# MisEty/X-SLAM

Hardware: AMD Instinct MI355X
Metric: fps XKinectFusion 512^3 TSDF 640x480 CSFD @1/2/4/8 GPU; HBM GB/s on integrate (higher is better)
Workload: dtype f32 (complex<f32> CSFD)

## Files before the change

include/xslam_amd_pipeline.h:

```cpp
#ifndef XSLAM_AMD_PIPELINE_H
#define XSLAM_AMD_PIPELINE_H
#include <stddef.h>
#include <stdint.h>
#ifdef __cplusplus
extern "C" {
#endif

int xs_host_double_complex_table(int op, long n, const float *a, const float *b, float *out);
int xs_host_complex_table(int op, long n, const float *a, const float *b, float *out);

int xs_flat_yaml_get(const char *yaml_text, const char *key, char *out, int capacity);

void xs_kf_set_stream(void *stream);
void *xs_kf_create(const char *yaml_text);
void *xs_kf_create_sharded(const char *yaml_text, int rank, int count, void (*collective)(void *user, int op, void *dev_ptr, long n),
                           void *user);
void xs_kf_shard_planes(void *kf, int *owned2, int *stored2);
void xs_kf_destroy(void *kf);
void xs_kf_set_gt_poses(void *kf, int n, const float *c2w32);
int xs_kf_process_frame(void *kf, const uint16_t *depth_dev, size_t step_bytes);
void xs_kf_hint_next_frame(void *kf, const uint16_t *depth_dev, size_t step_bytes);
int xs_kf_process_frame_host(void *kf, const uint16_t *depth_host);
uint16_t *xs_kf_ingest_buffer(void *kf);
void xs_kf_get_camera2volume(void *kf, float *out32);
int xs_kf_gauss_newton_terms(void *kf, const uint16_t *depth_dev, size_t step_bytes, const float *c2v32, double *out29);
int xs_kf_relocalize(void *kf, const uint16_t *depth_dev, size_t step_bytes, float *c2v32, int iterations, float damping, double *loss_out);
int xs_kf_relocalize_batch(void *kf, int frames, const uint16_t *const *depth_dev, size_t step_bytes, float *c2v32xF, int iterations, float damping,
                           double *loss_out, int *ok_out);
int xs_kf_pose_hessian_terms(void *kf, const uint16_t *depth_dev, size_t step_bytes, const float *c2v32, double *out29);
int xs_kf_relocalize_newton(void *kf, const uint16_t *depth_dev, size_t step_bytes, float *c2v32, int iterations, float damping, double *loss_out,
                            int *fallbacks_out);
int xs_kf_relocalize_newton_batch(void *kf, int frames, const uint16_t *const *depth_dev, size_t step_bytes, float *c2v32xF, int iterations,
                                  float damping, double *loss_out, int *ok_out, int *fallbacks_out);
int xs_host_newton_seeded_poses(const float *c2v32, float *R36x21, float *t12x21);
int xs_host_newton_step(const double *s29, double damping, float *c2v32);
int xs_kf_score_poses(void *kf, const uint16_t *depth_dev, size_t step_bytes, int poses, const float *c2v32xP, double *out2xP);
int xs_kf_relocalize_global(void *kf, const uint16_t *depth_dev, size_t step_bytes, int poses, const float *c2v32xP, int keep, int iterations,
                            float damping, float *best_c2v32, double *report8);
struct xs_view_opts;
int xs_kf_score_views(void *kf, int poses, const float *c2v32xP, const struct xs_view_opts *opts, int min_weight, unsigned *out4xP);
int xs_kf_next_best_view(void *kf, int poses, const float *c2v32xP, const struct xs_view_opts *opts, int min_weight, unsigned min_hits,
                         unsigned *out4xP);
int xs_kf_clearance_field(void *kf, int max_radius_vox, int unknown_blocks, int min_weight, uint16_t *host_out);
int xs_kf_reachable(void *kf, const float *start_c2v32_or_null, float radius_m, int snap_vox, int unknown_blocks, int min_weight, int P, const float *c2v32xP,
                    unsigned char *reachable, unsigned short *clear2);
int xs_kf_next_reachable_view(void *kf, int poses, const float *c2v32xP, const struct xs_view_opts *opts, int min_weight, unsigned min_hits, unsigned *out4xP,
                              float radius_m, int snap_vox, int unknown_blocks, unsigned char *reachable);
int xs_kf_travel(void *kf, const float *start_c2v32_or_null, float radius_m, int snap_vox, int unknown_blocks, int min_weight, float max_travel_m, int P,
                 const float *c2v32xP, unsigned char *reachable, unsigned short *clear2, unsigned short *travel3);
int xs_kf_path_to(void *kf, const float *start_c2v32_or_null, float radius_m, int snap_vox, int unknown_blocks, int min_weight, float max_travel_m,
                  const float *target_c2v32, int capacity, int *voxels3, float *points3, int *needed_out);
int xs_kf_next_view_by_travel(void *kf, int poses, const float *c2v32xP, const struct xs_view_opts *opts, int min_weight, unsigned min_hits, unsigned *out4xP,
                              float radius_m, int snap_vox, int unknown_blocks, float max_travel_m, float bias_m, unsigned short *travel3_out);
int xs_kf_frontiers(void *kf, int cell, unsigned long long min_size, int min_weight, int capacity, unsigned long long *records8, int *count_out);
int xs_kf_propose_views(void *kf, float radius_m, int start_snap_vox, int unknown_blocks, int min_weight, int cell, unsigned long long min_size,
                        int views_per_cluster, float standoff_m, int snap_vox, int capacity, float *c2v32xP_out, int *cluster_out, int *count_out);
long long xs_kf_relocalization_index_voxels(void *kf);
long long xs_kf_export_point_cloud(void *kf, int max_buffer, float *points_host, float *normals_host);
long long xs_kf_export_ply(void *kf, int max_buffer, const char *filename);
long long xs_kf_export_mesh(void *kf, int min_weight, long long vertex_capacity, long long triangle_capacity, float *vertices_host,
                            float *normals_host, float *vertex_im_host, unsigned long long *edge_keys_host, int *triangles_host,
                            long long *triangle_count, int *has_im);
long long xs_kf_export_mesh_ply(void *kf, const char *filename);
void xs_kf_synchronize(void *kf);

int xs_kf_frame_id(void *kf);
int xs_kf_num_poses(void *kf);
void xs_kf_get_world2camera(void *kf, int idx, float *out32);
float xs_kf_tranc_dist(void *kf);
long long xs_kf_last_updated_voxels(void *kf);
long long xs_kf_last_raycast_hits(void *kf);
int xs_kf_icp_log(void *kf, double *out, int capacity);

int xs_kf_download_volume(void *kf, float *value, int *weight, float *grad);
int xs_kf_download_map(void *kf, int which, int level, float *out);
void *xs_kf_volume_ptr(void *kf, int which, size_t *step_bytes);

void xs_kf_set_profiling(void *kf, int level);
void xs_kf_stage_times(void *kf, double *ms6, long long *calls6);
void xs_kf_cumulative_counters(void *kf, long long *updated, long long *hits);
void xs_kf_reset_stage_times(void *kf);
void xs_kf_icp_iteration_times(void *kf, double *us4, long long *calls4);
void xs_kf_tail_host_times(void *kf, double *us4, long long *frames);
void xs_kf_gn_times(void *kf, double *pass_us, long long *passes, double *kernel_ms, long long *kernel_calls, int reset);
void xs_kf_gn_poll_times(void *kf, double *poll_us, long long *poll_passes, int reset);
void xs_kf_set_gn_post_pose(void *kf, int on);
void xs_kf_debug_set_icp_sequence(void *kf, unsigned long long v);
void xs_kf_debug_fail_icp_iteration(void *kf, int n);
void xs_kf_debug_post_delay(void *kf, int min_us, int max_us);
void xs_kf_rebuild_sign_map(void *kf);
long long xs_kf_composite_bytes(void *kf);
void xs_kf_list_cover_counts(void *kf, long long *counts4);

long long xs_kf_volume_generation(void *kf);
int xs_kf_save_checkpoint(void *kf, const char *path);
int xs_kf_load_checkpoint(void *kf, const char *path);
int xs_kf_save_tsdf_volume(void *kf, const char *path);

int xs_kf_merge_volume(void *kf, const float *src_value, const int *src_weight, const float *src_grad, size_t src_step, const int *src_res,
                       float src_voxel_size, float src_tranc_dist, const double *T16, int min_weight, unsigned long long *written);
int xs_kf_merge_map(void *kf, void *other_kf, const double *T16, int min_weight, unsigned long long *written);
int xs_kf_merge_checkpoint(void *kf, const char *path, const double *T16, int min_weight, unsigned long long *written);
int xs_host_merge_affine(const double *T16, double dst_voxel_size, double src_voxel_size, float *out12);
int xs_host_map_transform(const double *c2v_this16, const double *c2v_other16, double *T16);
int xs_host_merge_tile_box(const float *xform12, const int *lo3, const int *hi3, const int *src_res, int *box6);

int xs_kf_align_map(void *kf, void *other_kf, const double *T16xN, int N, int iterations, double damping, int min_weight, float max_residual,
                    double *T16_out, double *report8, double *loss_history);
int xs_kf_align_checkpoint(void *kf, const char *path, const double *T16xN, int N, int iterations, double damping, int min_weight, float max_residual,
                           double *T16_out, double *report8, double *loss_history);
int xs_host_align_seeded_maps(const double *T16, double vs_this, double vs_other, float *out144);
int xs_host_align_step(const double *s29, double damping, double *T16);

void *xs_refshape_create(const char *yaml_text);
void xs_refshape_destroy(void *rs);
int xs_refshape_process_frame_host(void *rs, const uint16_t *depth_host);
int xs_refshape_process_frame(void *rs, const uint16_t *depth_dev, size_t step_bytes);
int xs_refshape_frame_id(void *rs);
void xs_refshape_get_world2camera(void *rs, int idx, float *out32);
int xs_refshape_download_volume(void *rs, float *value, int *weight, float *grad);
int xs_refshape_download_map(void *rs, int which, int level, float *out);
int xs_refshape_icp_log(void *rs, double *out, int capacity);
int xs_refshape_hessian(const uint16_t *depth_dev, size_t depth_step, int rows, int cols, const float *intr4, const int *res3, float voxel_size,
                        const float *Rv2c36, const float *tv2c12, float tranc_dist, const float *gt_dev, int with_volumes, float *out4,
                        float *volumes_host);
int xs_refshape_loss(const uint16_t *depth_dev, size_t depth_step, int rows, int cols, const float *intr4, const int *res3, float voxel_size,
                     const float *Rv2c9, const float *tv2c3, float tranc_dist, const float *gt_dev, int with_volumes, float *out2,
                     float *volumes_host);

#ifdef __cplusplus
}
#endif
#endif
```

x-slam_amd/host/device_array.hpp:

```cpp
#pragma once
#include "kernel_containers.hpp"
#include <atomic>
#include <cstdio>
#include <cstdlib>
#include <hip/hip_runtime_api.h>
#include <hip/hip_vector_types.h>
#include <utility>
#include <vector>

namespace xs_host {
inline void safe_call(hipError_t err, const char *msg = nullptr) {
    if (hipSuccess != err) {
        printf("HIP error(%s): %s\n", msg ? msg : "", hipGetErrorString(err));
        exit(-1);
    }
}
inline hipStream_t &current_stream() { static thread_local hipStream_t s = nullptr; return s; }
}
#define hipSafeCall(e) xs_host::safe_call((e), #e)

class DeviceMemory {
public:
    DeviceMemory() : data_(nullptr), sizeBytes_(0), refcount_(nullptr) {}
    ~DeviceMemory() { release(); }
    DeviceMemory(size_t sizeBytes_arg) : data_(nullptr), sizeBytes_(0), refcount_(nullptr) { create(sizeBytes_arg); }
    DeviceMemory(void *ptr_arg, size_t sizeBytes_arg) : data_(ptr_arg), sizeBytes_(sizeBytes_arg), refcount_(nullptr) {}
    DeviceMemory(const DeviceMemory &o) : data_(o.data_), sizeBytes_(o.sizeBytes_), refcount_(o.refcount_) { if (refcount_) refcount_->fetch_add(1); }
    DeviceMemory &operator=(const DeviceMemory &o) {
        if (this != &o) {
            if (o.refcount_) o.refcount_->fetch_add(1);
            release();
            data_ = o.data_; sizeBytes_ = o.sizeBytes_; refcount_ = o.refcount_;
        }
        return *this;
    }
    void create(size_t sizeBytes_arg) {
        if (sizeBytes_arg == sizeBytes_) return;
        if (sizeBytes_arg > 0) {
            if (data_) release();
            sizeBytes_ = sizeBytes_arg;
            hipSafeCall(hipMalloc(&data_, sizeBytes_));
            refcount_ = new std::atomic<int>(1);
        }
    }
    void release() {
        if (refcount_ && refcount_->fetch_sub(1) == 1) {
            delete refcount_;
            hipSafeCall(hipFree(data_));
        }
        data_ = nullptr; sizeBytes_ = 0; refcount_ = nullptr;
    }
    void copyTo(DeviceMemory &other) const {
        if (empty()) other.release();
        else {
            other.create(sizeBytes_);
            hipSafeCall(hipMemcpyAsync(other.data_, data_, sizeBytes_, hipMemcpyDeviceToDevice, xs_host::current_stream()));
            hipSafeCall(hipStreamSynchronize(xs_host::current_stream()));
        }
    }
    void upload(const void *host_ptr_arg, size_t sizeBytes_arg) {
        create(sizeBytes_arg);
        hipSafeCall(hipMemcpyAsync(data_, host_ptr_arg, sizeBytes_, hipMemcpyHostToDevice, xs_host::current_stream()));
        hipSafeCall(hipStreamSynchronize(xs_host::current_stream()));
    }
    bool upload(const void *host_ptr_arg, std::size_t device_begin_byte_offset, std::size_t num_bytes) {
        if (device_begin_byte_offset + num_bytes > sizeBytes_) return false;
        hipSafeCall(hipMemcpyAsync((char *)data_ + device_begin_byte_offset, host_ptr_arg, num_bytes, hipMemcpyHostToDevice, xs_host::current_stream()));
        hipSafeCall(hipStreamSynchronize(xs_host::current_stream()));
        return true;
    }
    void download(void *host_ptr_arg) const {
        hipSafeCall(hipMemcpyAsync(host_ptr_arg, data_, sizeBytes_, hipMemcpyDeviceToHost, xs_host::current_stream()));
        hipSafeCall(hipStreamSynchronize(xs_host::current_stream()));
    }
    bool download(void *host_ptr_arg, std::size_t device_begin_byte_offset, std::size_t num_bytes) const {
        if (device_begin_byte_offset + num_bytes > sizeBytes_) return false;
        hipSafeCall(hipMemcpyAsync(host_ptr_arg, (const char *)data_ + device_begin_byte_offset, num_bytes, hipMemcpyDeviceToHost, xs_host::current_stream()));
        hipSafeCall(hipStreamSynchronize(xs_host::current_stream()));
        return true;
    }
    void swap(DeviceMemory &o) { std::swap(data_, o.data_); std::swap(sizeBytes_, o.sizeBytes_); std::swap(refcount_, o.refcount_); }
    template <class T> T *ptr() { return (T *)data_; }
    template <class T> const T *ptr() const { return (const T *)data_; }
    template <class U> operator PtrSz<U>() const { PtrSz<U> r; r.data = (U *)ptr<U>(); r.size = sizeBytes_ / sizeof(U); return r; }
    bool empty() const { return !data_; }
    size_t sizeBytes() const { return sizeBytes_; }

private:
    void *data_;
    std::size_t sizeBytes_;
    std::atomic<int> *refcount_;
};

class DeviceMemory2D {
public:
    DeviceMemory2D() : data_(nullptr), step_(0), colsBytes_(0), rows_(0), refcount_(nullptr) {}
    ~DeviceMemory2D() { release(); }
    DeviceMemory2D(int rows_arg, int colsBytes_arg) : data_(nullptr), step_(0), colsBytes_(0), rows_(0), refcount_(nullptr) { create(rows_arg, colsBytes_arg); }
    DeviceMemory2D(int rows_arg, int colsBytes_arg, void *data_arg, size_t step_arg)
        : data_(data_arg), step_(step_arg), colsBytes_(colsBytes_arg), rows_(rows_arg), refcount_(nullptr) {}
    DeviceMemory2D(const DeviceMemory2D &o) : data_(o.data_), step_(o.step_), colsBytes_(o.colsBytes_), rows_(o.rows_), refcount_(o.refcount_) {
        if (refcount_) refcount_->fetch_add(1);
    }
    DeviceMemory2D &operator=(const DeviceMemory2D &o) {
        if (this != &o) {
            if (o.refcount_) o.refcount_->fetch_add(1);
            release();
            colsBytes_ = o.colsBytes_; rows_ = o.rows_; data_ = o.data_; step_ = o.step_; refcount_ = o.refcount_;
        }
        return *this;
    }
    void create(int rows_arg, int colsBytes_arg) {
        if (colsBytes_ == colsBytes_arg && rows_ == rows_arg) return;
        if (rows_arg > 0 && colsBytes_arg > 0) {
            if (data_) release();
            colsBytes_ = colsBytes_arg; rows_ = rows_arg;
            step_ = ((size_t)colsBytes_ + 255) / 256 * 256;
            hipSafeCall(hipMalloc(&data_, step_ * (size_t)rows_));
            refcount_ = new std::atomic<int>(1);
        }
    }
    void release() {
        if (refcount_ && refcount_->fetch_sub(1) == 1) {
            delete refcount_;
            hipSafeCall(hipFree(data_));
        }
        colsBytes_ = 0; rows_ = 0; data_ = nullptr; step_ = 0; refcount_ = nullptr;
    }
    void copyTo(DeviceMemory2D &other) const {
        if (empty()) other.release();
        else {
            other.create(rows_, colsBytes_);
            hipSafeCall(hipMemcpy2DAsync(other.data_, other.step_, data_, step_, colsBytes_, rows_, hipMemcpyDeviceToDevice, xs_host::current_stream()));
            hipSafeCall(hipStreamSynchronize(xs_host::current_stream()));
        }
    }
    void upload(const void *host_ptr_arg, std::size_t host_step_arg, int rows_arg, int colsBytes_arg) {
        create(rows_arg, colsBytes_arg);
        hipSafeCall(hipMemcpy2DAsync(data_, step_, host_ptr_arg, host_step_arg, colsBytes_, rows_, hipMemcpyHostToDevice, xs_host::current_stream()));
        hipSafeCall(hipStreamSynchronize(xs_host::current_stream()));
    }
    void download(void *host_ptr_arg, std::size_t host_step_arg) const {
        hipSafeCall(hipMemcpy2DAsync(host_ptr_arg, host_step_arg, data_, step_, colsBytes_, rows_, hipMemcpyDeviceToHost, xs_host::current_stream()));
        hipSafeCall(hipStreamSynchronize(xs_host::current_stream()));
    }
    void swap(DeviceMemory2D &o) {
        std::swap(data_, o.data_); std::swap(step_, o.step_); std::swap(colsBytes_, o.colsBytes_); std::swap(rows_, o.rows_); std::swap(refcount_, o.refcount_);
    }
    template <class T> T *ptr(int y_arg = 0) { return (T *)((char *)data_ + y_arg * step_); }
    template <class T> const T *ptr(int y_arg = 0) const { return (const T *)((const char *)data_ + y_arg * step_); }
    template <class U> operator PtrStep<U>() const { PtrStep<U> r; r.data = (U *)ptr<U>(); r.step = step_; return r; }
    template <class U> operator PtrStepSz<U>() const {
        PtrStepSz<U> r; r.data = (U *)ptr<U>(); r.step = step_; r.cols = colsBytes_ / sizeof(U); r.rows = rows_; return r;
    }
    bool empty() const { return !data_; }
    int colsBytes() const { return colsBytes_; }
    int rows() const { return rows_; }
    size_t step() const { return step_; }

private:
    void *data_;
    std::size_t step_;
    int colsBytes_;
    int rows_;
    std::atomic<int> *refcount_;
};

template <class T>
class DeviceArray : public DeviceMemory {
public:
    using type = T;
    enum { elem_size = sizeof(T) };
    DeviceArray() {}
    DeviceArray(std::size_t size) : DeviceMemory(size * elem_size) {}
    DeviceArray(T *ptr, std::size_t size) : DeviceMemory(ptr, size * elem_size) {}
    DeviceArray(const DeviceArray &other) : DeviceMemory(other) {}
    DeviceArray &operator=(const DeviceArray &other) { DeviceMemory::operator=(other); return *this; }
    void create(std::size_t size) { DeviceMemory::create(size * elem_size); }
    void release() { DeviceMemory::release(); }
    void copyTo(DeviceArray &other) const { DeviceMemory::copyTo(other); }
    void upload(const T *host_ptr, std::size_t size) { DeviceMemory::upload(host_ptr, size * elem_size); }
    bool upload(const T *host_ptr, std::size_t device_begin_offset, std::size_t num_elements) {
        return DeviceMemory::upload(host_ptr, device_begin_offset * elem_size, num_elements * elem_size);
    }
    void download(T *host_ptr) const { DeviceMemory::download(host_ptr); }
    bool download(T *host_ptr, std::size_t device_begin_offset, std::size_t num_elements) const {
        return DeviceMemory::download(host_ptr, device_begin_offset * elem_size, num_elements * elem_size);
    }
    template <class A> void upload(const std::vector<T, A> &data) { upload(&data[0], data.size()); }
    template <typename A> void download(std::vector<T, A> &data) const { data.resize(size()); if (!data.empty()) download(&data[0]); }
    void swap(DeviceArray &other_arg) { DeviceMemory::swap(other_arg); }
    T *ptr() { return DeviceMemory::ptr<T>(); }
    const T *ptr() const { return DeviceMemory::ptr<T>(); }
    operator T *() { return ptr(); }
    operator const T *() const { return ptr(); }
    std::size_t size() const { return sizeBytes() / elem_size; }
};

template <class T>
class DeviceArray2D : public DeviceMemory2D {
public:
    using type = T;
    enum { elem_size = sizeof(T) };
    DeviceArray2D() {}
    DeviceArray2D(int rows, int cols) : DeviceMemory2D(rows, cols * elem_size) {}
    DeviceArray2D(int rows, int cols, void *data, std::size_t stepBytes) : DeviceMemory2D(rows, cols * elem_size, data, stepBytes) {}
    DeviceArray2D(const DeviceArray2D &other) : DeviceMemory2D(other) {}
    DeviceArray2D &operator=(const DeviceArray2D &other) { DeviceMemory2D::operator=(other); return *this; }
    void create(int rows, int cols) { DeviceMemory2D::create(rows, cols * elem_size); }
    void release() { DeviceMemory2D::release(); }
    void copyTo(DeviceArray2D &other) const { DeviceMemory2D::copyTo(other); }
    void upload(const void *host_ptr, std::size_t host_step, int rows, int cols) { DeviceMemory2D::upload(host_ptr, host_step, rows, cols * elem_size); }
    void download(void *host_ptr, std::size_t host_step) const { DeviceMemory2D::download(host_ptr, host_step); }
    void swap(DeviceArray2D &other_arg) { DeviceMemory2D::swap(other_arg); }
    template <class A> void upload(const std::vector<T, A> &data, int cols) { upload(&data[0], cols * elem_size, data.size() / cols, cols); }
    template <class A> void download(std::vector<T, A> &data, int &elem_step) const {
        elem_step = cols();
        data.resize(cols() * rows());
        if (!data.empty()) download(&data[0], colsBytes());
    }
    T *ptr(int y = 0) { return DeviceMemory2D::ptr<T>(y); }
    const T *ptr(int y = 0) const { return DeviceMemory2D::ptr<T>(y); }
    operator T *() { return ptr(); }
    operator const T *() const { return ptr(); }
    int cols() const { return DeviceMemory2D::colsBytes() / elem_size; }
    int rows() const { return DeviceMemory2D::rows(); }
    std::size_t elem_step() const { return DeviceMemory2D::step() / elem_size; }
};
```

x-slam_amd/host/xs_launchers.hpp:

```cpp
#pragma once
#include "../../include/xslam_amd.h"
#include "xs_types.hpp"
#include "host_algebra.hpp"

namespace xs_host {
inline void check_rc(int rc, const char *what) {
    if (rc != 0) {
        printf("HIP error(%s): %s\n", what, xs_last_error());
        exit(-1);
    }
}
inline void sync() { hipSafeCall(hipStreamSynchronize(current_stream())); }
struct Scratch {
    DeviceArray<unsigned char> icp_ws, reduce_ws, integrate_ws;
    DeviceArray<double> sums;
    DeviceArray<float> ray_ws;
    static Scratch &get() { static thread_local Scratch s; return s; }
    void *icp() {
        if (icp_ws.size() != xs_icp_workspace_bytes()) {
            icp_ws.create(xs_icp_workspace_bytes());
            check_rc(xs_icp_workspace_init(icp_ws.ptr(), current_stream()), "icp workspace");
        }
        return icp_ws.ptr();
    }
    void *integrate(const int *res) {
        const size_t bytes = xs_integrate_workspace_bytes(res, res[2]);
        if (integrate_ws.size() != bytes) integrate_ws.create(bytes);
        return integrate_ws.ptr();
    }
    float *ray(int rows, int cols) { if (ray_ws.size() != (size_t)rows * cols) ray_ws.create((size_t)rows * cols); return ray_ws.ptr(); }
    void *reduce() {
        if (reduce_ws.size() != xs_tsdf_reduce_workspace_bytes()) {
            reduce_ws.create(xs_tsdf_reduce_workspace_bytes());
            check_rc(xs_tsdf_reduce_workspace_init(reduce_ws.ptr(), current_stream()), "reduce workspace");
        }
        return reduce_ws.ptr();
    }
    double *sum_buf() { if (sums.size() != 64) sums.create(64); return sums.ptr(); }
};
}

inline void initVolume(PtrStep<short> , PtrStep<float> value_volume,
                       PtrStep<int> weight_volume, PtrStep<float> grad_volume, const int3 &volume_resolution) {
    const int res[3] = {volume_resolution.x, volume_resolution.y, volume_resolution.z};
    xs_host::check_rc(xs_init_volume(value_volume.data, weight_volume.data, grad_volume.data, value_volume.step, res, 0, res[2],
                                     xs_host::current_stream()), "initVolume");
    xs_host::sync();
}

inline void integrateTsdfVolume(const PtrStepSz<ushort> &depth, const Intr &intr, int max_weight, const int3 &volume_resolution,
                                float voxel_size, const MatS33 &Rv2c, const devComplex3 &tv2c, const devComplex3 & ,
                                float tranc_dist, PtrStep<float> value_volume, PtrStep<int> weight_volume, PtrStep<float> grad_volume,
                                DeviceArray2D<float> &depthScaled, int , float threshold = 0.0f, float  = 0.0f,
                                unsigned long long *updated_dev = nullptr, bool synchronise = true) {
    depthScaled.create(depth.rows, depth.cols);
    const int res[3] = {volume_resolution.x, volume_resolution.y, volume_resolution.z};
    hipStream_t st = xs_host::current_stream();
    xs_host::check_rc(xs_scale_depth(depth.data, depth.step, depth.rows, depth.cols, depthScaled.ptr(), depthScaled.step(), st), "scaleDepth");
    xs_host::check_rc(xs_integrate_scaled(depthScaled.ptr(), depthScaled.step(), depth.rows, depth.cols, &intr.fx, max_weight, res, voxel_size,
                                          &Rv2c.data[0].x.re, &tv2c.x.re, tranc_dist, value_volume.data, weight_volume.data, grad_volume.data,
                                          value_volume.step, threshold, 0, res[2], updated_dev, nullptr, xs_host::Scratch::get().integrate(res), st),
                      "integrateTsdfVolume");
    if (synchronise) xs_host::sync();
}

inline void raycast(const Intr &intr, const MatS33 &Rc2v, const devComplex3 &tc2v, const MatS33 &Rv2w, const devComplex3 &tv2w,
                    float tranc_dist, const int3 &volume_resolution, float voxel_size, const PtrStep<float> &value_volume,
                    const PtrStep<float> &grad_volume, MapArr &vmap, MapArr &nmap, unsigned long long *hits_dev = nullptr,
                    float *workspace = nullptr, xs_raycast_opts *opts = nullptr) {
    const int res[3] = {volume_resolution.x, volume_resolution.y, volume_resolution.z};
    xs_host::check_rc(xs_raycast_ex(&intr.fx, &Rc2v.data[0].x.re, &tc2v.x.re, &Rv2w.data[0].x.re, &tv2w.x.re, tranc_dist, res, voxel_size,
                                    value_volume.data, grad_volume.data, value_volume.step, &vmap.ptr()->re, &nmap.ptr()->re, vmap.step(),
                                    vmap.rows() / 3, vmap.cols(), hits_dev, workspace ? workspace : xs_host::Scratch::get().ray(vmap.rows() / 3, vmap.cols()), opts,
                                    xs_host::current_stream()), "raycast");
}

inline void estimateCombined(const MatS33 &Rcurr, const devComplex3 &tcurr, const MapArr &vmap_curr, const MapArr &nmap_curr,
                             const MatS33 &Rprev_inv, const devComplex3 &tprev, const Intr &intr, const MapArr &vmap_g_prev,
                             const MapArr &nmap_g_prev, float distThres, float angleThres, DeviceArray2D<devComplexICP> & ,
                             DeviceArray<devComplexICP> & , hostComplexICP *matrixA_host, hostComplexICP *vectorB_host,
                             long long *inliers = nullptr) {
    auto &S = xs_host::Scratch::get();
    xs_host::check_rc(xs_estimate_combined(&Rcurr.data[0].x.re, &tcurr.x.re, &vmap_curr.ptr()->re, &nmap_curr.ptr()->re,
                                           &Rprev_inv.data[0].x.re, &tprev.x.re, &intr.fx, &vmap_g_prev.ptr()->re, &nmap_g_prev.ptr()->re,
                                           vmap_curr.step(), vmap_curr.rows() / 3, vmap_curr.cols(), distThres, angleThres, S.icp(),
                                           nullptr , reinterpret_cast<double *>(matrixA_host), reinterpret_cast<double *>(vectorB_host),
                                           inliers, xs_host::current_stream()), "estimateCombined");
}

inline void bilateralFilter(const DeviceArray2D<ushort> &src, MapArr &dst) {
    xs_host::check_rc(xs_bilateral_filter(src.ptr(), src.step(), src.rows(), src.cols(), &dst.ptr()->re, dst.step(), xs_host::current_stream()), "bilateralFilter");
}
inline void pyrDown(const MapArr &src, MapArr &dst) {
    dst.create(src.rows() / 2, src.cols() / 2);
    xs_host::check_rc(xs_pyr_down(&src.ptr()->re, src.step(), src.rows(), src.cols(), &dst.ptr()->re, dst.step(), xs_host::current_stream()), "pyrDown");
}
inline void createVMap(const Intr &intr, const MapArr &depth, MapArr &vmap) {
    vmap.create(depth.rows() * 3, depth.cols());
    xs_host::check_rc(xs_create_vmap(&intr.fx, &depth.ptr()->re, depth.step(), depth.rows(), depth.cols(), &vmap.ptr()->re, vmap.step(), xs_host::current_stream()), "createVMap");
}
inline void createNMap(const MapArr &vmap, MapArr &nmap) {
    nmap.create(vmap.rows(), vmap.cols());
    xs_host::check_rc(xs_create_nmap(&vmap.ptr()->re, &nmap.ptr()->re, vmap.step(), vmap.rows() / 3, vmap.cols(), xs_host::current_stream()), "createNMap");
}
inline void resizeVMap(const MapArr &input, MapArr &output, bool synchronise = true) {
    output.create((input.rows() / 3 / 2) * 3, input.cols() / 2);
    xs_host::check_rc(xs_resize_vmap(&input.ptr()->re, input.step(), input.rows() / 3, input.cols(), &output.ptr()->re, output.step(), xs_host::current_stream()), "resizeVMap");
    if (synchronise) xs_host::sync();
}
inline void resizeNMap(const MapArr &input, MapArr &output, bool synchronise = true) {
    output.create((input.rows() / 3 / 2) * 3, input.cols() / 2);
    xs_host::check_rc(xs_resize_nmap(&input.ptr()->re, input.step(), input.rows() / 3, input.cols(), &output.ptr()->re, output.step(), xs_host::current_stream()), "resizeNMap");
    if (synchronise) xs_host::sync();
}

inline float4 ComputeLocalTsdf_hessian(const PtrStepSz<ushort> &depth, const Intr &intr, DeviceArray2D<float> &depthScaled,
                                        const int3 &volume_resolution, float voxel_size, const MatD33 &Rv2c, const devDComplex3 &tv2c,
                                        float tranc_dist, float , float , DeviceArray<float> &gt_vec,
                                        DeviceArray<float> &real_vec, DeviceArray<float> &grad_vec, DeviceArray<float> &hessian_vec,
                                        DeviceArray<int> &count_vec) {
    depthScaled.create(depth.rows, depth.cols);
    const int res[3] = {volume_resolution.x, volume_resolution.y, volume_resolution.z};
    auto &S = xs_host::Scratch::get();
    hipStream_t st = xs_host::current_stream();
    xs_host::check_rc(xs_scale_depth(depth.data, depth.step, depth.rows, depth.cols, depthScaled.ptr(), depthScaled.step(), st), "scaleDepth");
    const bool vols = !real_vec.empty() && !grad_vec.empty() && !hessian_vec.empty() && !count_vec.empty();
    xs_host::check_rc(xs_compute_local_tsdf_hessian(depthScaled.ptr(), depthScaled.step(), depth.rows, depth.cols, &intr.fx, res, voxel_size,
                                                    &Rv2c.data[0].x.re_re, &tv2c.x.re_re, tranc_dist, gt_vec.ptr(),
                                                    vols ? real_vec.ptr() : nullptr, vols ? grad_vec.ptr() : nullptr,
                                                    vols ? hessian_vec.ptr() : nullptr, vols ? count_vec.ptr() : nullptr, 0, res[2],
                                                    S.reduce(), S.sum_buf(), st), "ComputeLocalTsdf_hessian");
    double h[4];
    hipSafeCall(hipMemcpyAsync(h, S.sum_buf(), sizeof(h), hipMemcpyDeviceToHost, st));
    xs_host::sync();
    return float4{(float)h[0], (float)h[1], (float)h[2], (float)h[3]};
}
inline float2 ComputeLocalTsdf_loss(const PtrStepSz<ushort> &depth, const Intr &intr, DeviceArray2D<float> &depthScaled,
                                     const int3 &volume_resolution, float voxel_size, const Mat33 &Rv2c, const float3 &tv2c,
                                     float tranc_dist, float , float , DeviceArray<float> &gt_vec,
                                     DeviceArray<float> &real_vec, DeviceArray<int> &count_vec) {
    depthScaled.create(depth.rows, depth.cols);
    const int res[3] = {volume_resolution.x, volume_resolution.y, volume_resolution.z};
    auto &S = xs_host::Scratch::get();
    hipStream_t st = xs_host::current_stream();
    xs_host::check_rc(xs_scale_depth(depth.data, depth.step, depth.rows, depth.cols, depthScaled.ptr(), depthScaled.step(), st), "scaleDepth");
    const bool vols = !real_vec.empty() && !count_vec.empty();
    xs_host::check_rc(xs_compute_local_tsdf_loss(depthScaled.ptr(), depthScaled.step(), depth.rows, depth.cols, &intr.fx, res, voxel_size,
                                                 &Rv2c.data[0].x, &tv2c.x, tranc_dist, gt_vec.ptr(), vols ? real_vec.ptr() : nullptr,
                                                 vols ? count_vec.ptr() : nullptr, 0, res[2], S.reduce(), S.sum_buf(), st), "ComputeLocalTsdf_loss");
    double h[2];
    hipSafeCall(hipMemcpyAsync(h, S.sum_buf(), sizeof(h), hipMemcpyDeviceToHost, st));
    xs_host::sync();
    return float2{(float)h[0], (float)h[1]};
}

inline size_t extractPoints(const PtrStep<float> &value_volume, const PtrStep<int> & , const PtrStep<float> & ,
                            const int3 &volume_resolution, float voxel_size, PtrSz<float3> output, int zs0 = 0, int z0 = 0, int z1 = -1) {
    const int res[3] = {volume_resolution.x, volume_resolution.y, volume_resolution.z};
    static thread_local DeviceArray<unsigned char> ws;
    if (ws.size() < xs_extract_workspace_bytes(res)) ws.create(xs_extract_workspace_bytes(res));
    size_t count = 0;
    xs_host::check_rc(xs_extract_points(value_volume.data, value_volume.step, res, voxel_size, zs0, z0, z1 < 0 ? res[2] - 1 : z1,
                                        reinterpret_cast<float *>(output.data), output.size, ws.ptr(), &count, nullptr, xs_host::current_stream()),
                      "extractPoints");
    return count;
}
inline void extractNormals(const PtrStep<float> &value_volume, const PtrStep<int> & , const PtrStep<float> & ,
                           const int3 &volume_resolution, float voxel_size, PtrSz<float3> points, PtrSz<float3> normal, int zs0 = 0, int zs1 = -1) {
    const int res[3] = {volume_resolution.x, volume_resolution.y, volume_resolution.z};
    xs_host::check_rc(xs_extract_normals(value_volume.data, value_volume.step, res, voxel_size, zs0, zs1 < 0 ? res[2] : zs1,
                                         reinterpret_cast<const float *>(points.data), points.size, reinterpret_cast<float *>(normal.data),
                                         xs_host::current_stream()), "extractNormals");
    xs_host::sync();
}
```

x-slam_amd/pipeline.py:

```python
import collections
import ctypes as C
import os

import numpy as np

from . import capi

_HERE = os.path.dirname(os.path.abspath(__file__))
LIB_PATH = os.path.join(_HERE, "libxslam_host.so")
if not os.path.exists(LIB_PATH):
    raise ImportError(f"{LIB_PATH} not found: run __graft_entry__.build() (make -C x-slam_amd/host). There is no CPU fallback.")
_lib = C.CDLL(LIB_PATH)

_vp, _sz = C.c_void_p, C.c_size_t
_f32p, _f64p, _i32p = C.POINTER(C.c_float), C.POINTER(C.c_double), C.POINTER(C.c_int)
COLLECTIVE_CB = C.CFUNCTYPE(None, C.c_void_p, C.c_int, C.c_void_p, C.c_long)
_SIGS = {
    "xs_kf_create_sharded": (_vp, [C.c_char_p, C.c_int, C.c_int, COLLECTIVE_CB, _vp]),
    "xs_kf_shard_planes": (None, [_vp, _i32p, _i32p]),
    "xs_host_double_complex_table": (C.c_int, [C.c_int, C.c_long, _f32p, _f32p, _f32p]),
    "xs_host_complex_table": (C.c_int, [C.c_int, C.c_long, _f32p, _f32p, _f32p]),
    "xs_flat_yaml_get": (C.c_int, [C.c_char_p, C.c_char_p, C.c_char_p, C.c_int]),
    "xs_kf_set_stream": (None, [_vp]),
    "xs_kf_create": (_vp, [C.c_char_p]),
    "xs_kf_destroy": (None, [_vp]),
    "xs_kf_set_gt_poses": (None, [_vp, C.c_int, _f32p]),
    "xs_kf_process_frame": (C.c_int, [_vp, _vp, _sz]),
    "xs_kf_process_frame_host": (C.c_int, [_vp, _vp]),
    "xs_kf_ingest_buffer": (_vp, [_vp]),
    "xs_kf_get_camera2volume": (None, [_vp, _f32p]),
    "xs_kf_gauss_newton_terms": (C.c_int, [_vp, _vp, _sz, _f32p, _f64p]),
    "xs_kf_relocalize": (C.c_int, [_vp, _vp, _sz, _f32p, C.c_int, C.c_float, _f64p]),
    "xs_kf_relocalize_batch": (C.c_int, [_vp, C.c_int, C.POINTER(_vp), _sz, _f32p, C.c_int, C.c_float, _f64p, _i32p]),
    "xs_kf_pose_hessian_terms": (C.c_int, [_vp, _vp, _sz, _f32p, _f64p]),
    "xs_kf_relocalize_newton": (C.c_int, [_vp, _vp, _sz, _f32p, C.c_int, C.c_float, _f64p, _i32p]),
    "xs_kf_relocalize_newton_batch": (C.c_int, [_vp, C.c_int, C.POINTER(_vp), _sz, _f32p, C.c_int, C.c_float, _f64p, _i32p, _i32p]),
    "xs_host_newton_seeded_poses": (C.c_int, [_f32p, _f32p, _f32p]),
    "xs_host_newton_step": (C.c_int, [_f64p, C.c_double, _f32p]),
    "xs_kf_score_poses": (C.c_int, [_vp, _vp, _sz, C.c_int, _f32p, _f64p]),
    "xs_kf_relocalize_global": (C.c_int, [_vp, _vp, _sz, C.c_int, _f32p, C.c_int, C.c_int, C.c_float, _f32p, _f64p]),
    "xs_kf_score_views": (C.c_int, [_vp, C.c_int, _f32p, C.POINTER(capi.ViewOpts), C.c_int, C.POINTER(C.c_uint)]),
    "xs_kf_next_best_view": (C.c_int, [_vp, C.c_int, _f32p, C.POINTER(capi.ViewOpts), C.c_int, C.c_uint, C.POINTER(C.c_uint)]),
    "xs_kf_clearance_field": (C.c_int, [_vp, C.c_int, C.c_int, C.c_int, C.POINTER(C.c_uint16)]),
    "xs_kf_reachable": (C.c_int, [_vp, _f32p, C.c_float, C.c_int, C.c_int, C.c_int, C.c_int, _f32p, C.POINTER(C.c_ubyte), C.POINTER(C.c_uint16)]),
    "xs_kf_next_reachable_view": (C.c_int, [_vp, C.c_int, _f32p, C.POINTER(capi.ViewOpts), C.c_int, C.c_uint, C.POINTER(C.c_uint), C.c_float, C.c_int,
                                            C.c_int, C.POINTER(C.c_ubyte)]),
    "xs_kf_travel": (C.c_int, [_vp, _f32p, C.c_float, C.c_int, C.c_int, C.c_int, C.c_float, C.c_int, _f32p, C.POINTER(C.c_ubyte), C.POINTER(C.c_uint16),
                               C.POINTER(C.c_uint16)]),
    "xs_kf_path_to": (C.c_int, [_vp, _f32p, C.c_float, C.c_int, C.c_int, C.c_int, C.c_float, _f32p, C.c_int, _i32p, _f32p, _i32p]),
    "xs_kf_next_view_by_travel": (C.c_int, [_vp, C.c_int, _f32p, C.POINTER(capi.ViewOpts), C.c_int, C.c_uint, C.POINTER(C.c_uint), C.c_float, C.c_int,
                                            C.c_int, C.c_float, C.c_float, C.POINTER(C.c_uint16)]),
    "xs_kf_frontiers": (C.c_int, [_vp, C.c_int, C.c_ulonglong, C.c_int, C.c_int, C.POINTER(C.c_uint64), _i32p]),
    "xs_kf_propose_views": (C.c_int, [_vp, C.c_float, C.c_int, C.c_int, C.c_int, C.c_int, C.c_ulonglong, C.c_int, C.c_float, C.c_int, C.c_int, _f32p, _i32p,
                                      _i32p]),
    "xs_kf_relocalization_index_voxels": (C.c_longlong, [_vp]),
    "xs_kf_export_point_cloud": (C.c_longlong, [_vp, C.c_int, _f32p, _f32p]),
    "xs_kf_export_ply": (C.c_longlong, [_vp, C.c_int, C.c_char_p]),
    "xs_kf_export_mesh": (C.c_longlong, [_vp, C.c_int, C.c_longlong, C.c_longlong, _f32p, _f32p, _f32p, C.POINTER(C.c_uint64), _i32p,
                                         C.POINTER(C.c_longlong), _i32p]),
    "xs_kf_export_mesh_ply": (C.c_longlong, [_vp, C.c_char_p]),
    "xs_kf_synchronize": (None, [_vp]),
    "xs_kf_frame_id": (C.c_int, [_vp]),
    "xs_kf_num_poses": (C.c_int, [_vp]),
    "xs_kf_get_world2camera": (None, [_vp, C.c_int, _f32p]),
    "xs_kf_tranc_dist": (C.c_float, [_vp]),
    "xs_kf_last_updated_voxels": (C.c_longlong, [_vp]),
    "xs_kf_last_raycast_hits": (C.c_longlong, [_vp]),
    "xs_kf_icp_log": (C.c_int, [_vp, _f64p, C.c_int]),
    "xs_kf_download_volume": (C.c_int, [_vp, _f32p, _i32p, _f32p]),
    "xs_kf_download_map": (C.c_int, [_vp, C.c_int, C.c_int, _f32p]),
    "xs_kf_volume_ptr": (_vp, [_vp, C.c_int, C.POINTER(_sz)]),
    "xs_kf_set_profiling": (None, [_vp, C.c_int]),
    "xs_kf_stage_times": (None, [_vp, _f64p, C.POINTER(C.c_longlong)]),
    "xs_kf_reset_stage_times": (None, [_vp]),
    "xs_kf_icp_iteration_times": (None, [_vp, _f64p, C.POINTER(C.c_longlong)]),
    "xs_kf_tail_host_times": (None, [_vp, _f64p, C.POINTER(C.c_longlong)]),
    "xs_kf_set_gn_post_pose": (None, [_vp, C.c_int]),
    "xs_kf_gn_poll_times": (None, [_vp, _f64p, C.POINTER(C.c_longlong), C.c_int]),
    "xs_kf_gn_times": (None, [_vp, _f64p, C.POINTER(C.c_longlong), _f64p, C.POINTER(C.c_longlong), C.c_int]),
    "xs_kf_debug_set_icp_sequence": (None, [_vp, C.c_ulonglong]),
    "xs_kf_debug_fail_icp_iteration": (None, [_vp, C.c_int]),
    "xs_kf_debug_post_delay": (None, [_vp, C.c_int, C.c_int]),
    "xs_kf_composite_bytes": (C.c_longlong, [_vp]),
    "xs_kf_rebuild_sign_map": (None, [_vp]),
    "xs_kf_hint_next_frame": (None, [_vp, _vp, _sz]),
    "xs_kf_list_cover_counts": (None, [_vp, C.POINTER(C.c_longlong)]),
    "xs_kf_cumulative_counters": (None, [_vp, C.POINTER(C.c_longlong), C.POINTER(C.c_longlong)]),
    "xs_kf_volume_generation": (C.c_longlong, [_vp]),
    "xs_kf_save_checkpoint": (C.c_int, [_vp, C.c_char_p]),
    "xs_kf_load_checkpoint": (C.c_int, [_vp, C.c_char_p]),
    "xs_kf_save_tsdf_volume": (C.c_int, [_vp, C.c_char_p]),
    "xs_kf_merge_volume": (C.c_int, [_vp, _vp, _vp, _vp, _sz, _i32p, C.c_float, C.c_float, _f64p, C.c_int, C.POINTER(C.c_ulonglong)]),
    "xs_kf_merge_map": (C.c_int, [_vp, _vp, _f64p, C.c_int, C.POINTER(C.c_ulonglong)]),
    "xs_kf_merge_checkpoint": (C.c_int, [_vp, C.c_char_p, _f64p, C.c_int, C.POINTER(C.c_ulonglong)]),
    "xs_host_merge_affine": (C.c_int, [_f64p, C.c_double, C.c_double, _f32p]),
    "xs_host_map_transform": (C.c_int, [_f64p, _f64p, _f64p]),
    "xs_host_merge_tile_box": (C.c_int, [_f32p, _i32p, _i32p, _i32p, _i32p]),
    "xs_kf_align_map": (C.c_int, [_vp, _vp, _f64p, C.c_int, C.c_int, C.c_double, C.c_int, C.c_float, _f64p, _f64p, _f64p]),
    "xs_kf_align_checkpoint": (C.c_int, [_vp, C.c_char_p, _f64p, C.c_int, C.c_int, C.c_double, C.c_int, C.c_float, _f64p, _f64p, _f64p]),
    "xs_host_align_seeded_maps": (C.c_int, [_f64p, C.c_double, C.c_double, _f32p]),
    "xs_host_align_step": (C.c_int, [_f64p, C.c_double, _f64p]),
    "xs_refshape_create": (_vp, [C.c_char_p]),
    "xs_refshape_destroy": (None, [_vp]),
    "xs_refshape_process_frame_host": (C.c_int, [_vp, _vp]),
    "xs_refshape_process_frame": (C.c_int, [_vp, _vp, _sz]),
    "xs_refshape_frame_id": (C.c_int, [_vp]),
    "xs_refshape_get_world2camera": (None, [_vp, C.c_int, _f32p]),
    "xs_refshape_download_volume": (C.c_int, [_vp, _f32p, _i32p, _f32p]),
    "xs_refshape_download_map": (C.c_int, [_vp, C.c_int, C.c_int, _f32p]),
    "xs_refshape_icp_log": (C.c_int, [_vp, _f64p, C.c_int]),
    "xs_refshape_hessian": (C.c_int, [_vp, _sz, C.c_int, C.c_int, _f32p, _i32p, C.c_float, _f32p, _f32p, C.c_float, _vp, C.c_int, _f32p, _f32p]),
    "xs_refshape_loss": (C.c_int, [_vp, _sz, C.c_int, C.c_int, _f32p, _i32p, C.c_float, _f32p, _f32p, C.c_float, _vp, C.c_int, _f32p, _f32p]),
}
for _n, (_r, _a) in _SIGS.items():
    _f = getattr(_lib, _n)
    _f.restype, _f.argtypes = _r, _a

STAGES = ("surface", "icp", "scale", "integrate", "raycast", "resize")
MAPS = {"depths_curr": 0, "vmaps_curr": 1, "nmaps_curr": 2, "vmaps_g_prev": 3, "nmaps_g_prev": 4}


def yaml_text(params: dict) -> str:
    out = []
    for k, v in params.items():
        if isinstance(v, bool):
            v = "true" if v else "false"
        elif isinstance(v, float):
            v = repr(float(np.float32(v))) if abs(v) < 1e-3 and v != 0 else repr(v)
        out.append(f"{k}: {v}")
    return "\n".join(out) + "\n"


HDC_OPS = {"add": 0, "sub": 1, "mul": 2, "div": 3, "sqrt": 4, "abs": 5, "exp": 6, "log": 7, "sin": 8, "cos": 9, "pow": 10, "f1": 11,
           "conj": 12, "norm": 13, "cmp": 14}


def host_double_complex(op, a, b=None):
    a = np.ascontiguousarray(a, dtype=np.float32).reshape(-1, 4)
    b = a if b is None else np.ascontiguousarray(b, dtype=np.float32).reshape(-1, 4)
    out = np.empty_like(a)
    rc = _lib.xs_host_double_complex_table(HDC_OPS[op], a.shape[0], a.ctypes.data_as(_f32p), b.ctypes.data_as(_f32p), out.ctypes.data_as(_f32p))
    if rc != 0:
        raise ValueError("bad op")
    return out


def host_complex(op_code, a, b=None):
    a = np.ascontiguousarray(a, dtype=np.float32).reshape(-1, 2)
    b = a if b is None else np.ascontiguousarray(b, dtype=np.float32).reshape(-1, 2)
    out = np.empty_like(a)
    rc = _lib.xs_host_complex_table(int(op_code), a.shape[0], a.ctypes.data_as(_f32p), b.ctypes.data_as(_f32p), out.ctypes.data_as(_f32p))
    if rc != 0:
        raise ValueError("bad op")
    return out


def host_newton_seeded_poses(c2v):
    m = np.ascontiguousarray(c2v, dtype=np.float32).reshape(32)
    R, t = np.zeros((21, 3, 3, 4), np.float32), np.zeros((21, 3, 4), np.float32)
    _lib.xs_host_newton_seeded_poses(m.ctypes.data_as(_f32p), R.ctypes.data_as(_f32p), t.ctypes.data_as(_f32p))
    return R, t


def host_newton_step(s29, damping, c2v):
    s = np.ascontiguousarray(s29, dtype=np.float64).reshape(29)
    m = np.ascontiguousarray(c2v, dtype=np.float32).reshape(32).copy()
    rc = _lib.xs_host_newton_step(s.ctypes.data_as(_f64p), float(damping), m.ctypes.data_as(_f32p))
    return rc == 0, m.reshape(4, 4, 2)


def _real44(m):
    a = np.asarray(m, dtype=np.float64)
    if a.shape == (4, 4, 2):
        a = a[..., 0]
    return np.ascontiguousarray(a.reshape(4, 4))


def merge_affine(T, dst_voxel_size, src_voxel_size):
    t = _real44(T)
    out = np.zeros(12, np.float32)
    if _lib.xs_host_merge_affine(t.ctypes.data_as(_f64p), float(dst_voxel_size), float(src_voxel_size), out.ctypes.data_as(_f32p)) != 0:
        raise ValueError("merge_affine: an input is not finite, or a voxel size is not positive")
    return out


def map_transform(c2v_this, c2v_other):
    a, b = _real44(c2v_this), _real44(c2v_other)
    out = np.zeros((4, 4), np.float64)
    _lib.xs_host_map_transform(a.ctypes.data_as(_f64p), b.ctypes.data_as(_f64p), out.ctypes.data_as(_f64p))
    return out


def align_seeded_maps(T, vs_this, vs_other):
    t = _real44(T)
    out = np.zeros((6, 12, 2), np.float32)
    if _lib.xs_host_align_seeded_maps(t.ctypes.data_as(_f64p), float(vs_this), float(vs_other), out.ctypes.data_as(_f32p)) != 0:
        raise ValueError("align_seeded_maps: an input is not finite, or a voxel size is not positive")
    return out


def align_step(s29, damping, T):
    s = np.ascontiguousarray(s29, dtype=np.float64).reshape(29)
    t = _real44(T).copy()
    rc = _lib.xs_host_align_step(s.ctypes.data_as(_f64p), float(damping), t.ctypes.data_as(_f64p))
    return rc == 0, t


def merge_tile_box(xform12, lo, hi, src_res):
    m = np.ascontiguousarray(xform12, np.float32).reshape(12)
    l, h, s = (np.ascontiguousarray(a, np.int32).reshape(3) for a in (lo, hi, src_res))
    box = np.zeros(6, np.int32)
    rc = _lib.xs_host_merge_tile_box(m.ctypes.data_as(_f32p), l.ctypes.data_as(_i32p), h.ctypes.data_as(_i32p), s.ctypes.data_as(_i32p), box.ctypes.data_as(_i32p))
    return (box[:3].copy(), box[3:].copy()) if rc == 1 else None


def _halton(i, base):
    f, r = 1.0, 0.0
    while i > 0:
        f /= base
        r += f * (i % base)
        i //= base
    return r


def _se3_exp(xi):
    v, w = np.asarray(xi[:3], np.float64), np.asarray(xi[3:], np.float64)
    th = float(np.linalg.norm(w))
    K = np.array([[0.0, -w[2], w[1]], [w[2], 0.0, -w[0]], [-w[1], w[0], 0.0]])
    if th < 1e-12:
        R, V = np.eye(3) + K, np.eye(3) + K
    else:
        R = np.eye(3) + np.sin(th) / th * K + (1 - np.cos(th)) / th ** 2 * K @ K
        V = np.eye(3) + (1 - np.cos(th)) / th ** 2 * K + (th - np.sin(th)) / th ** 3 * K @ K
    T = np.eye(4)
    T[:3, :3], T[:3, 3] = R, V @ v
    return T


POSE_CANDIDATE_PRIMES = (2, 3, 5, 7, 11, 13)


def pose_candidates(center_c2v, box_t, box_r, n):
    c = np.asarray(center_c2v, np.float64)
    c = c[..., 0] if c.ndim == 3 else c
    assert c.shape == (4, 4)
    out = np.zeros((int(n), 4, 4, 2), np.float32)
    for i in range(int(n)):
        u = np.array([2.0 * _halton(i + 1, b) - 1.0 for b in POSE_CANDIDATE_PRIMES])
        out[i, ..., 0] = c @ _se3_exp(np.concatenate([u[:3] * float(box_t), u[3:] * float(box_r)]))
    return out


def flat_yaml_get(text, key):
    buf = C.create_string_buffer(1024)
    n = _lib.xs_flat_yaml_get(text.encode(), key.encode(), buf, 1024)
    return None if n < 0 else buf.value.decode()


def set_stream(stream):
    _lib.xs_kf_set_stream(None if stream is None else (stream.cuda_stream if hasattr(stream, "cuda_stream") else int(stream)))


class Mesh(collections.namedtuple("Mesh", "vertices vertex_im normals triangles edge_keys")):
    """A triangle mesh of the TSDF (KinectFusion.export_mesh): numpy arrays, vertices in ascending edge key."""


class KinectFusion:

    def __init__(self, params, gt_poses=None):
        text = params if isinstance(params, str) else yaml_text(params)
        self.cfg = {}
        for line in text.splitlines():
            if ":" in line:
                k, v = line.split(":", 1)
                self.cfg[k.strip()] = v.split("#")[0].strip()
        self.h = _lib.xs_kf_create(text.encode())
        if not self.h:
            raise ValueError("xs_kf_create failed (missing config key, or a retired one set?)")
        self.res = [int(self.cfg[f"tsdf_size_{a}"]) for a in "xyz"]
        self.width, self.height = int(self.cfg["depth_width"]), int(self.cfg["depth_height"])
        if gt_poses is not None:
            g = np.ascontiguousarray(gt_poses, dtype=np.float32).reshape(-1, 32)
            _lib.xs_kf_set_gt_poses(self.h, g.shape[0], g.ctypes.data_as(_f32p))

    def close(self):
        if getattr(self, "h", None) and _lib is not None:
            _lib.xs_kf_destroy(self.h)
            self.h = None

    def __del__(self):
        self.close()

    def process_frame(self, depth_dev, step_bytes=None):
        ptr = depth_dev if isinstance(depth_dev, int) else depth_dev.data_ptr()
        step = step_bytes if step_bytes is not None else self.width * 2
        return _lib.xs_kf_process_frame(self.h, ptr, step)

    def hint_next_frame(self, depth_dev, step_bytes=None):
        _lib.xs_kf_hint_next_frame(self.h, depth_dev.data_ptr(), step_bytes or self.width * 2)

    def process_frame_host(self, depth_u16):
        d = np.ascontiguousarray(depth_u16, dtype=np.uint16)
        return _lib.xs_kf_process_frame_host(self.h, d.ctypes.data)

    def ingest_buffer(self):
        ptr = _lib.xs_kf_ingest_buffer(self.h)
        n = self.width * self.height
        return np.ctypeslib.as_array((C.c_uint16 * n).from_address(ptr)).reshape(self.height, self.width)

    def camera2volume(self):
        out = np.zeros(32, np.float32)
        _lib.xs_kf_get_camera2volume(self.h, out.ctypes.data_as(_f32p))
        return out.reshape(4, 4, 2)

    def gauss_newton_terms(self, depth_dev, c2v):
        m = np.ascontiguousarray(c2v, dtype=np.float32).reshape(32)
        out = np.zeros(29, np.float64)
        ok = _lib.xs_kf_gauss_newton_terms(self.h, depth_dev.data_ptr(), self.width * 2, m.ctypes.data_as(_f32p), out.ctypes.data_as(_f64p))
        return out if ok == 1 else None

    def pose_hessian_terms(self, depth_dev, c2v):
        m = np.ascontiguousarray(c2v, dtype=np.float32).reshape(32)
        out = np.zeros(29, np.float64)
        ok = _lib.xs_kf_pose_hessian_terms(self.h, depth_dev.data_ptr(), self.width * 2, m.ctypes.data_as(_f32p), out.ctypes.data_as(_f64p))
        return out if ok == 1 else None

    def pose_hessian(self, depth_dev, c2v):
        s = self.pose_hessian_terms(depth_dev, c2v)
        if s is None:
            return None
        H = np.zeros((6, 6))
        H[np.triu_indices(6)] = s[:21]
        H = H + np.triu(H, 1).T
        return H, s[21:27].copy(), float(s[27]), int(s[28])

    def relocalize(self, depth_dev, c2v, iterations=5, damping=1e-3, method="gauss_newton"):
        m = np.ascontiguousarray(c2v, dtype=np.float32).reshape(32).copy()
        hist = np.zeros(iterations + 1, np.float64)
        if method == "newton":
            fb = C.c_int(0)
            ok = _lib.xs_kf_relocalize_newton(self.h, depth_dev.data_ptr(), self.width * 2, m.ctypes.data_as(_f32p), iterations, damping,
                                              hist.ctypes.data_as(_f64p), C.cast(C.byref(fb), _i32p))
            return ok == 1, m.reshape(4, 4, 2), hist, int(fb.value)
        if method != "gauss_newton":
            raise ValueError(f"relocalize: unknown method {method!r}")
        ok = _lib.xs_kf_relocalize(self.h, depth_dev.data_ptr(), self.width * 2, m.ctypes.data_as(_f32p), iterations, damping,
                                   hist.ctypes.data_as(_f64p))
        return ok == 1, m.reshape(4, 4, 2), hist

    def relocalize_batch(self, depths, c2vs, iterations=5, damping=1e-3, method="gauss_newton"):
        F = len(depths)
        m = np.ascontiguousarray(c2vs, dtype=np.float32).reshape(F * 32).copy()
        hist = np.zeros((F, iterations + 1), np.float64)
        ok = np.zeros(F, np.int32)
        P = (_vp * max(F, 1))(*[d if isinstance(d, int) else d.data_ptr() for d in depths])
        if method == "newton":
            fb = np.zeros(max(F, 1), np.int32)
            n = _lib.xs_kf_relocalize_newton_batch(self.h, F, P, self.width * 2, m.ctypes.data_as(_f32p), iterations, damping,
                                                   hist.ctypes.data_as(_f64p), ok.ctypes.data_as(_i32p), fb.ctypes.data_as(_i32p))
            if n < 0:
                raise ValueError("xs_kf_relocalize_newton_batch: bad arguments")
            return ok == 1, m.reshape(F, 4, 4, 2), hist, fb[:F]
        if method != "gauss_newton":
            raise ValueError(f"relocalize_batch: unknown method {method!r}")
        n = _lib.xs_kf_relocalize_batch(self.h, F, P, self.width * 2, m.ctypes.data_as(_f32p), iterations, damping, hist.ctypes.data_as(_f64p),
                                        ok.ctypes.data_as(_i32p))
        if n < 0:
            raise ValueError("xs_kf_relocalize_batch: bad arguments")
        return ok == 1, m.reshape(F, 4, 4, 2), hist

    def score_poses(self, depth_dev, c2vs):
        m = np.ascontiguousarray(c2vs, dtype=np.float32).reshape(-1)
        P = m.size // 32
        assert m.size == 32 * P
        out = np.zeros((max(P, 1), 2), np.float64)
        rc = _lib.xs_kf_score_poses(self.h, depth_dev.data_ptr(), self.width * 2, P, m.ctypes.data_as(_f32p), out.ctypes.data_as(_f64p))
        if rc != 1:
            raise ValueError("xs_kf_score_poses: bad arguments" if rc < 0 else "xs_kf_score_poses: no volume")
        return out[:P, 0].copy(), out[:P, 1].copy()

    def relocalize_global(self, depth_dev, candidates, keep=8, iterations=10, damping=1e-3):
        m = np.ascontiguousarray(candidates, dtype=np.float32).reshape(-1)
        P = m.size // 32
        assert m.size == 32 * P and P > 0
        best = m[:32].copy()
        rep = np.zeros(8, np.float64)
        rc = _lib.xs_kf_relocalize_global(self.h, depth_dev.data_ptr(), self.width * 2, P, m.ctypes.data_as(_f32p), int(keep), int(iterations),
                                          float(damping), best.ctypes.data_as(_f32p), rep.ctypes.data_as(_f64p))
        if rc < 0:
            raise ValueError("xs_kf_relocalize_global: bad arguments")
        report = dict(index=int(rep[0]), S_before=float(rep[1]), S_after=float(rep[2]), sum_loss_after=float(rep[3]), count_after=float(rep[4]),
                      refined_ok=int(rep[5]), index_voxels=int(rep[6]))
        return rc == 1, best.reshape(4, 4, 2), report

    @staticmethod
    def _view_call(name, rc, bad):
        if rc == -2:
            raise capi.XsError(f"{name}: not available in shard mode (occlusion along a ray is not additive over z-slabs)")
        if rc == bad:
            raise ValueError(f"{name}: bad arguments or options")

    def score_views(self, c2vs, rays=(80, 60), t_near=0.2, t_far=5.0, step=None, min_weight=1):
        m = np.ascontiguousarray(c2vs, dtype=np.float32).reshape(-1)
        P = m.size // 32
        assert m.size == 32 * P
        out = np.zeros((max(P, 1), 4), np.uint32)
        opts = capi.view_opts(rays, t_near, t_far, step)
        rc = _lib.xs_kf_score_views(self.h, P, m.ctypes.data_as(_f32p), C.byref(opts), int(min_weight), out.ctypes.data_as(C.POINTER(C.c_uint)))
        self._view_call("xs_kf_score_views", rc, -1)
        if rc != 1:
            raise ValueError("xs_kf_score_views: no volume")
        return out[:P].copy()

    def next_best_view(self, candidates, min_hits=None, rays=(80, 60), t_near=0.2, t_far=5.0, step=None, min_weight=1):
        m = np.ascontiguousarray(candidates, dtype=np.float32).reshape(-1)
        P = m.size // 32
        assert m.size == 32 * P
        if min_hits is None:
            min_hits = int(rays[0]) * int(rays[1]) // 4
        out = np.zeros((max(P, 1), 4), np.uint32)
        opts = capi.view_opts(rays, t_near, t_far, step)
        rc = _lib.xs_kf_next_best_view(self.h, P, m.ctypes.data_as(_f32p), C.byref(opts), int(min_weight), int(min_hits),
                                       out.ctypes.data_as(C.POINTER(C.c_uint)))
        self._view_call("xs_kf_next_best_view", rc, -3)
        return int(rc), out[:P].copy()

    def clearance_field(self, max_radius_vox=8, unknown_blocks=True, min_weight=1):
        out = np.zeros((self.res[2], self.res[1], self.res[0]), np.uint16)
        rc = _lib.xs_kf_clearance_field(self.h, int(max_radius_vox), int(bool(unknown_blocks)), int(min_weight), out.ctypes.data_as(C.POINTER(C.c_uint16)))
        self._reach_call("xs_kf_clearance_field", rc, -1)
        if rc != 1:
            raise ValueError("xs_kf_clearance_field: no volume")
        return out

    @staticmethod
    def _reach_call(name, rc, bad):
        if rc == -2:
            raise capi.XsError(f"{name}: not available in shard mode (distance and connectivity are not additive over z-slabs)")
        if rc == bad:
            raise ValueError(f"{name}: bad arguments or options")

    def reachable(self, c2vs, radius_m, start=None, snap_vox=4, unknown_blocks=True, min_weight=1):
        m = np.ascontiguousarray(c2vs, dtype=np.float32).reshape(-1)
        P = m.size // 32
        assert m.size == 32 * P
        flags, clear2 = np.zeros(max(P, 1), np.uint8), np.zeros(max(P, 1), np.uint16)
        s = None if start is None else np.ascontiguousarray(start, dtype=np.float32).reshape(32)
        rc = _lib.xs_kf_reachable(self.h, None if s is None else s.ctypes.data_as(_f32p), float(radius_m), int(snap_vox), int(bool(unknown_blocks)),
                                  int(min_weight), P, m.ctypes.data_as(_f32p), flags.ctypes.data_as(C.POINTER(C.c_ubyte)),
                                  clear2.ctypes.data_as(C.POINTER(C.c_uint16)))
        self._reach_call("xs_kf_reachable", rc, -1)
        if rc != 1:
            raise ValueError("xs_kf_reachable: no volume")
        return flags[:P].astype(bool), clear2[:P].copy()

    def next_reachable_view(self, candidates, radius_m, min_hits=None, rays=(80, 60), t_near=0.2, t_far=5.0, step=None, min_weight=1, snap_vox=4,
                            unknown_blocks=True):
        m = np.ascontiguousarray(candidates, dtype=np.float32).reshape(-1)
        P = m.size // 32
        assert m.size == 32 * P
        if min_hits is None:
            min_hits = int(rays[0]) * int(rays[1]) // 4
        out, flags = np.zeros((max(P, 1), 4), np.uint32), np.zeros(max(P, 1), np.uint8)
        opts = capi.view_opts(rays, t_near, t_far, step)
        rc = _lib.xs_kf_next_reachable_view(self.h, P, m.ctypes.data_as(_f32p), C.byref(opts), int(min_weight), int(min_hits),
                                            out.ctypes.data_as(C.POINTER(C.c_uint)), float(radius_m), int(snap_vox), int(bool(unknown_blocks)),
                                            flags.ctypes.data_as(C.POINTER(C.c_ubyte)))
        self._reach_call("xs_kf_next_reachable_view", rc, -3)
        return int(rc), out[:P].copy(), flags[:P].astype(bool)

    def _travel_m(self, units):
        vs = float(np.float32(float(self.cfg["tsdf_voxel_size"])))
        u = np.asarray(units, np.uint16)
        return np.where(u == capi.TRAVEL_NONE, np.inf, u.astype(np.float64) * vs / 3.0)

    def travel(self, c2vs, radius_m, start=None, snap_vox=4, unknown_blocks=True, min_weight=1, max_travel_m=None):
        m = np.ascontiguousarray(c2vs, dtype=np.float32).reshape(-1)
        P = m.size // 32
        assert m.size == 32 * P
        flags, clear2, cost = np.zeros(max(P, 1), np.uint8), np.zeros(max(P, 1), np.uint16), np.zeros(max(P, 1), np.uint16)
        s = None if start is None else np.ascontiguousarray(start, dtype=np.float32).reshape(32)
        rc = _lib.xs_kf_travel(self.h, None if s is None else s.ctypes.data_as(_f32p), float(radius_m), int(snap_vox), int(bool(unknown_blocks)),
                               int(min_weight), 0.0 if max_travel_m is None else float(max_travel_m), P, m.ctypes.data_as(_f32p),
                               flags.ctypes.data_as(C.POINTER(C.c_ubyte)), clear2.ctypes.data_as(C.POINTER(C.c_uint16)),
                               cost.ctypes.data_as(C.POINTER(C.c_uint16)))
        self._reach_call("xs_kf_travel", rc, -1)
        if rc != 1:
            raise ValueError("xs_kf_travel: no volume")
        return flags[:P].astype(bool), clear2[:P].copy(), self._travel_m(cost[:P])

    def path_to(self, c2v, radius_m, start=None, snap_vox=4, unknown_blocks=True, min_weight=1, max_travel_m=None, capacity=1024):
        t = np.ascontiguousarray(c2v, dtype=np.float32).reshape(32)
        s = None if start is None else np.ascontiguousarray(start, dtype=np.float32).reshape(32)
        capacity = max(int(capacity), 1)
        for _ in range(2):
            voxels, points, needed = np.zeros((capacity, 3), np.int32), np.zeros((capacity, 3), np.float32), C.c_int(0)
            rc = _lib.xs_kf_path_to(self.h, None if s is None else s.ctypes.data_as(_f32p), float(radius_m), int(snap_vox), int(bool(unknown_blocks)),
                                    int(min_weight), 0.0 if max_travel_m is None else float(max_travel_m), t.ctypes.data_as(_f32p), capacity,
                                    voxels.ctypes.data_as(_i32p), points.ctypes.data_as(_f32p), C.byref(needed))
            if rc != -4:
                break
            capacity = int(needed.value)
        self._reach_call("xs_kf_path_to", rc, -1)
        if rc < 0:
            raise capi.XsError(f"xs_kf_path_to: {rc}")
        return None if rc == 0 else (points[:rc].copy(), voxels[:rc].copy())

    def next_view_by_travel(self, candidates, radius_m, bias_m=0.5, min_hits=None, rays=(80, 60), t_near=0.2, t_far=5.0, step=None, min_weight=1,
                            snap_vox=4, unknown_blocks=True, max_travel_m=None):
        m = np.ascontiguousarray(candidates, dtype=np.float32).reshape(-1)
        P = m.size // 32
        assert m.size == 32 * P
        if min_hits is None:
            min_hits = int(rays[0]) * int(rays[1]) // 4
        out, cost = np.zeros((max(P, 1), 4), np.uint32), np.zeros(max(P, 1), np.uint16)
        opts = capi.view_opts(rays, t_near, t_far, step)
        rc = _lib.xs_kf_next_view_by_travel(self.h, P, m.ctypes.data_as(_f32p), C.byref(opts), int(min_weight), int(min_hits),
                                            out.ctypes.data_as(C.POINTER(C.c_uint)), float(radius_m), int(snap_vox), int(bool(unknown_blocks)),
                                            0.0 if max_travel_m is None else float(max_travel_m), float(bias_m), cost.ctypes.data_as(C.POINTER(C.c_uint16)))
        self._reach_call("xs_kf_next_view_by_travel", rc, -3)
        return int(rc), out[:P].copy(), self._travel_m(cost[:P])

    FRONTIER_DTYPE = np.dtype([("label", np.uint32), ("count", np.uint64), ("sum", np.uint64, 3), ("centroid", np.float32, 3), ("min", np.int32, 3),
                               ("max", np.int32, 3)])

    @staticmethod
    def _frontier_call(name, rc):
        if rc == -2:
            raise capi.XsError(f"{name}: not available in shard mode (neither connectivity nor a cluster is additive over z-slabs)")
        if rc == -1:
            raise ValueError(f"{name}: bad arguments or options")

    def frontiers(self, cell_vox=32, min_size=8, min_weight=1):
        capacity, n = 1024, C.c_int(0)
        for _ in range(2):
            rec = np.zeros((max(capacity, 1), capi.FRONTIER_RECORD_WORDS), np.uint64)
            rc = _lib.xs_kf_frontiers(self.h, int(cell_vox), int(min_size), int(min_weight), capacity, rec.ctypes.data_as(C.POINTER(C.c_uint64)), C.byref(n))
            if rc != -4:
                break
            capacity = int(n.value)
        self._frontier_call("xs_kf_frontiers", rc)
        if rc != 1:
            raise ValueError("xs_kf_frontiers: no volume" if rc == 0 else f"xs_kf_frontiers: {rc}")
        rec = rec[:n.value]
        out = np.zeros(len(rec), self.FRONTIER_DTYPE)
        out["label"], out["count"], out["sum"] = rec[:, 0], rec[:, 1], rec[:, 2:5]
        vs = np.float32(float(self.cfg["tsdf_voxel_size"]))
        q = (rec[:, 2:5].astype(np.float64) / np.maximum(rec[:, 1:2], 1).astype(np.float64)).astype(np.float32)
        out["centroid"] = (q + np.float32(0.5)) * vs
        for name, col in (("min", 5), ("max", 6)):
            out[name] = np.stack([(rec[:, col] >> np.uint64(s)) & np.uint64(0xFFFF) for s in (0, 16, 32)], axis=1).astype(np.int32)
        return out

    def propose_views(self, radius_m, views_per_cluster=6, standoff_m=1.0, cell_vox=32, min_size=8, snap_vox=4, start_snap_vox=4, unknown_blocks=True,
                      min_weight=1):
        capacity, n = 1024, C.c_int(0)
        for _ in range(2):
            m, idx = np.zeros((max(capacity, 1), 4, 4, 2), np.float32), np.zeros(max(capacity, 1), np.int32)
            rc = _lib.xs_kf_propose_views(self.h, float(radius_m), int(start_snap_vox), int(bool(unknown_blocks)), int(min_weight), int(cell_vox), int(min_size),
                                          int(views_per_cluster), float(standoff_m), int(snap_vox), capacity, m.ctypes.data_as(_f32p), idx.ctypes.data_as(_i32p),
                                          C.byref(n))
            if rc != -4:
                break
            capacity = int(n.value)
        self._frontier_call("xs_kf_propose_views", rc)
        if rc != 1:
            raise ValueError("xs_kf_propose_views: no volume" if rc == 0 else f"xs_kf_propose_views: {rc}")
        return m[:n.value].copy(), idx[:n.value].copy()

    def explore_step(self, radius_m, views_per_cluster=6, standoff_m=1.0, cell_vox=32, min_size=8, snap_vox=4, unknown_blocks=True, min_weight=1, bias_m=0.5,
                     min_hits=None, rays=(80, 60), t_near=0.2, t_far=5.0, step=None, max_travel_m=None):
        cands, cluster = self.propose_views(radius_m, views_per_cluster, standoff_m, cell_vox, min_size, snap_vox, snap_vox, unknown_blocks, min_weight)
        if len(cands) == 0:
            return None
        pick, counts, travel_m = self.next_view_by_travel(cands, radius_m, bias_m=bias_m, min_hits=min_hits, rays=rays, t_near=t_near, t_far=t_far, step=step,
                                                          min_weight=min_weight, snap_vox=snap_vox, unknown_blocks=unknown_blocks, max_travel_m=max_travel_m)
        if pick < 0:
            return None
        path = self.path_to(cands[pick], radius_m, snap_vox=snap_vox, unknown_blocks=unknown_blocks, min_weight=min_weight, max_travel_m=max_travel_m)
        return dict(index=pick, pose=cands[pick].copy(), cluster=int(cluster[pick]), counts=counts[pick].copy(), travel_m=float(travel_m[pick]), path=path)

    def relocalization_index_voxels(self):
        return int(_lib.xs_kf_relocalization_index_voxels(self.h))

    def export_point_cloud(self, max_buffer=1000000):
        p = np.zeros((max_buffer, 3), np.float32)
        nr = np.zeros((max_buffer, 3), np.float32)
        n = _lib.xs_kf_export_point_cloud(self.h, max_buffer, p.ctypes.data_as(_f32p), nr.ctypes.data_as(_f32p))
        return p[:n], nr[:n]

    def export_ply(self, filename, max_buffer=1000000):
        return _lib.xs_kf_export_ply(self.h, max_buffer, str(filename).encode())

    def export_mesh(self, min_weight=1):
        nt, has_im = C.c_longlong(0), C.c_int(0)
        nv = _lib.xs_kf_export_mesh(self.h, min_weight, 0, 0, None, None, None, None, None, C.byref(nt), C.byref(has_im))
        while True:
            cap_v, cap_t = nv, nt.value
            v, n, im = (np.zeros((cap_v, 3), np.float32) for _ in range(3))
            k = np.zeros(cap_v, np.uint64)
            t = np.zeros((cap_t, 3), np.int32)
            nv = _lib.xs_kf_export_mesh(self.h, min_weight, cap_v, cap_t, v.ctypes.data_as(_f32p), n.ctypes.data_as(_f32p), im.ctypes.data_as(_f32p),
                                        k.ctypes.data_as(C.POINTER(C.c_uint64)), t.ctypes.data_as(_i32p), C.byref(nt), C.byref(has_im))
            if nv <= cap_v and nt.value <= cap_t:
                return Mesh(v[:nv], im[:nv] if has_im.value else None, n[:nv], t[:nt.value], k[:nv])

    def export_mesh_ply(self, filename):
        return _lib.xs_kf_export_mesh_ply(self.h, str(filename).encode())

    def synchronize(self):
        _lib.xs_kf_synchronize(self.h)

    @property
    def frame_id(self):
        return _lib.xs_kf_frame_id(self.h)

    def num_poses(self):
        return _lib.xs_kf_num_poses(self.h)

    def world2camera(self, idx=-1):
        out = np.zeros(32, np.float32)
        _lib.xs_kf_get_world2camera(self.h, idx, out.ctypes.data_as(_f32p))
        return out.reshape(4, 4, 2)

    def tranc_dist(self):
        return _lib.xs_kf_tranc_dist(self.h)

    def last_U(self):
        return _lib.xs_kf_last_updated_voxels(self.h)

    def last_hits(self):
        return _lib.xs_kf_last_raycast_hits(self.h)

    def icp_log(self):
        n = _lib.xs_kf_icp_log(self.h, None, 0)
        out = np.zeros(n, np.float64)
        if n:
            _lib.xs_kf_icp_log(self.h, out.ctypes.data_as(_f64p), n)
        return out.reshape(-1, 55)

    def volume(self):
        n = self.res[0] * self.res[1] * self.res[2]
        v, w, g = np.zeros(n, np.float32), np.zeros(n, np.int32), np.zeros(n, np.float32)
        _lib.xs_kf_download_volume(self.h, v.ctypes.data_as(_f32p), w.ctypes.data_as(_i32p), g.ctypes.data_as(_f32p))
        return v, w, g

    def map(self, which, level):
        rows, cols = self.height >> level, self.width >> level
        planes = 1 if which == "depths_curr" else 3
        out = np.zeros((planes * rows, cols, 2), np.float32)
        rc = _lib.xs_kf_download_map(self.h, MAPS[which], level, out.ctypes.data_as(_f32p))
        assert rc == 0
        return out

    def volume_ptr(self, which):
        step = _sz(0)
        p = _lib.xs_kf_volume_ptr(self.h, {"value": 0, "weight": 1, "grad": 2}[which], C.byref(step))
        return p, step.value

    def set_profiling(self, level=2):
        _lib.xs_kf_set_profiling(self.h, 2 if level is True else int(level))

    def stage_times(self):
        ms = np.zeros(6, np.float64)
        calls = (C.c_longlong * 6)()
        _lib.xs_kf_stage_times(self.h, ms.ctypes.data_as(_f64p), calls)
        return {s: (float(ms[i]), int(calls[i])) for i, s in enumerate(STAGES)}

    def cumulative_counters(self):
        u, h = C.c_longlong(0), C.c_longlong(0)
        _lib.xs_kf_cumulative_counters(self.h, C.byref(u), C.byref(h))
        return u.value, h.value

    def reset_stage_times(self):
        _lib.xs_kf_reset_stage_times(self.h)

    def icp_iteration_times(self):
        us = np.zeros(4, np.float64)
        calls = (C.c_longlong * 4)()
        _lib.xs_kf_icp_iteration_times(self.h, us.ctypes.data_as(_f64p), calls)
        return {lv: (float(us[lv]), int(calls[lv])) for lv in range(4)}

    def tail_host_times(self):
        us = np.zeros(4, np.float64)
        n = C.c_longlong(0)
        _lib.xs_kf_tail_host_times(self.h, us.ctypes.data_as(_f64p), C.byref(n))
        k = max(int(n.value), 1)
        return {"frames": int(n.value), "sums_seen_to_integrate_entered": round(float(us[0]) / k, 2), "entered_to_launch_call": round(float(us[1]) / k, 2),
                "integrate_launch_call": round(float(us[2]) / k, 2), "launch_returned_to_raycast_launched": round(float(us[3]) / k, 2)}

    def gn_poll_times(self, reset=False):
        pu, n = C.c_double(0), C.c_longlong(0)
        _lib.xs_kf_gn_poll_times(self.h, C.byref(pu), C.byref(n), int(reset))
        return {"passes": int(n.value), "wait_us": pu.value / max(n.value, 1)}

    def set_gn_post_pose(self, on):
        _lib.xs_kf_set_gn_post_pose(self.h, int(bool(on)))

    def gn_times(self, reset=False):
        pu, km = C.c_double(0), C.c_double(0)
        n, kc = C.c_longlong(0), C.c_longlong(0)
        _lib.xs_kf_gn_times(self.h, C.byref(pu), C.byref(n), C.byref(km), C.byref(kc), int(reset))
        return {"passes": int(n.value), "pass_us": pu.value / max(n.value, 1), "kernel_calls": int(kc.value), "kernel_us": 1e3 * km.value / max(kc.value, 1)}

    def debug_set_icp_sequence(self, v):
        _lib.xs_kf_debug_set_icp_sequence(self.h, int(v))

    def debug_fail_icp_iteration(self, n):
        _lib.xs_kf_debug_fail_icp_iteration(self.h, int(n))

    def debug_post_delay(self, min_us, max_us):
        _lib.xs_kf_debug_post_delay(self.h, int(min_us), int(max_us))

    def composite_bytes(self):
        return int(_lib.xs_kf_composite_bytes(self.h))

    def list_cover_counts(self):
        c = (C.c_longlong * 4)()
        _lib.xs_kf_list_cover_counts(self.h, c)
        return {"neither": int(c[0]), "list_only": int(c[1]), "both": int(c[3])}

    def rebuild_sign_map(self):
        _lib.xs_kf_rebuild_sign_map(self.h)

    def volume_generation(self):
        return int(_lib.xs_kf_volume_generation(self.h))

    def save_checkpoint(self, path):
        _lib.xs_kf_save_checkpoint(self.h, path.encode())

    def load_checkpoint(self, path):
        return _lib.xs_kf_load_checkpoint(self.h, path.encode()) == 0

    def save_tsdf_volume(self, path):
        _lib.xs_kf_save_tsdf_volume(self.h, path.encode())

    @staticmethod
    def _merge_call(name, rc, written):
        if rc == -2:
            raise capi.XsError(f"{name}: not available in shard mode")
        if rc == -1:
            raise ValueError(f"{name}: bad arguments (T not finite, min_weight < 1, the volume itself as source, a bad file or another truncation distance)")
        if rc != 1:
            raise ValueError(f"{name}: no volume" if rc == 0 else f"{name}: {rc}")
        return int(written.value)

    def merge_map(self, other, T=None, min_weight=1):
        t = _real44(np.eye(4) if T is None else T)
        n = C.c_ulonglong(0)
        return self._merge_call("xs_kf_merge_map", _lib.xs_kf_merge_map(self.h, other.h, t.ctypes.data_as(_f64p), int(min_weight), C.byref(n)), n)

    def merge_checkpoint(self, path, T=None, min_weight=1):
        t = _real44(np.eye(4) if T is None else T)
        n = C.c_ulonglong(0)
        return self._merge_call("xs_kf_merge_checkpoint", _lib.xs_kf_merge_checkpoint(self.h, path.encode(), t.ctypes.data_as(_f64p), int(min_weight), C.byref(n)), n)

    def _align_call(self, name, source, T0, iterations, damping, min_weight, max_residual):
        t = np.asarray(np.eye(4) if T0 is None else T0, dtype=np.float64)
        t = np.ascontiguousarray(t.reshape(-1, 4, 4))
        iterations = int(iterations)
        out, report, hist = np.zeros((4, 4), np.float64), np.zeros(8, np.float64), np.zeros(max(iterations, 0) + 1, np.float64)
        rc = getattr(_lib, name)(self.h, source, t.ctypes.data_as(_f64p), t.shape[0], iterations, float(damping), int(min_weight), float(max_residual),
                                 out.ctypes.data_as(_f64p), report.ctypes.data_as(_f64p), hist.ctypes.data_as(_f64p))
        if rc == -2:
            raise capi.XsError(f"{name}: not available in shard mode")
        if rc == -1:
            raise ValueError(f"{name}: bad arguments (T not finite, iterations < 0, min_weight < 1, max_residual or damping out of range, the volume itself "
                             "as source, a bad file or another truncation distance)")
        if rc not in (0, 1):
            raise ValueError(f"{name}: {rc}")
        rep = {"start": int(report[0]), "count": int(report[1]), "sum_r2": float(report[2]), "loss": float(report[3]), "passes": int(report[4]),
               "ended_ok": int(report[5]), "band_voxels": int(report[6])}
        return rc == 1, (out if rc == 1 else t[0].copy()), rep, (hist.copy() if rc == 1 else hist[:0].copy())

    def align_map(self, other, T0=None, iterations=10, damping=1e-3, min_weight=1, max_residual=1.0):
        return self._align_call("xs_kf_align_map", other.h, T0, iterations, damping, min_weight, max_residual)

    def align_checkpoint(self, path, T0=None, iterations=10, damping=1e-3, min_weight=1, max_residual=1.0):
        return self._align_call("xs_kf_align_checkpoint", path.encode(), T0, iterations, damping, min_weight, max_residual)


class ReferenceCallShape:

    def __init__(self, params):
        text = params if isinstance(params, str) else yaml_text(params)
        cfg = {}
        for line in text.splitlines():
            if ":" in line:
                k, v = line.split(":", 1)
                cfg[k.strip()] = v.split("#")[0].strip()
        self.h = _lib.xs_refshape_create(text.encode())
        if not self.h:
            raise ValueError("xs_refshape_create failed (missing config key?)")
        self.res = [int(cfg[f"tsdf_size_{a}"]) for a in "xyz"]
        self.width, self.height = int(cfg["depth_width"]), int(cfg["depth_height"])

    def close(self):
        if getattr(self, "h", None) and _lib is not None:
            _lib.xs_refshape_destroy(self.h)
            self.h = None

    def __del__(self):
        self.close()

    def process_frame(self, depth_dev, step_bytes=None):
        ptr = depth_dev if isinstance(depth_dev, int) else depth_dev.data_ptr()
        return _lib.xs_refshape_process_frame(self.h, ptr, step_bytes if step_bytes is not None else self.width * 2)

    def process_frame_host(self, depth_u16):
        d = np.ascontiguousarray(depth_u16, dtype=np.uint16)
        return _lib.xs_refshape_process_frame_host(self.h, d.ctypes.data)

    @property
    def frame_id(self):
        return _lib.xs_refshape_frame_id(self.h)

    def world2camera(self, idx=-1):
        out = np.zeros(32, np.float32)
        _lib.xs_refshape_get_world2camera(self.h, idx, out.ctypes.data_as(_f32p))
        return out.reshape(4, 4, 2)

    def volume(self):
        n = self.res[0] * self.res[1] * self.res[2]
        v, w, g = np.zeros(n, np.float32), np.zeros(n, np.int32), np.zeros(n, np.float32)
        _lib.xs_refshape_download_volume(self.h, v.ctypes.data_as(_f32p), w.ctypes.data_as(_i32p), g.ctypes.data_as(_f32p))
        return v, w, g

    def map(self, which, level):
        rows, cols = self.height >> level, self.width >> level
        planes = 1 if which == "depths_curr" else 3
        out = np.zeros((planes * rows, cols, 2), np.float32)
        assert _lib.xs_refshape_download_map(self.h, MAPS[which], level, out.ctypes.data_as(_f32p)) == 0
        return out

    def icp_log(self):
        n = _lib.xs_refshape_icp_log(self.h, None, 0)
        out = np.zeros(n, np.float64)
        if n:
            _lib.xs_refshape_icp_log(self.h, out.ctypes.data_as(_f64p), n)
        return out.reshape(-1, 54)


def reference_tsdf_hessian(depth_dev, rows, cols, intr4, res, voxel_size, R_dual, t_dual, tranc_dist, gt_dev, with_volumes=False):
    k = np.ascontiguousarray(intr4, np.float32)
    r3 = np.ascontiguousarray(res, np.int32)
    R = np.ascontiguousarray(R_dual, np.float32).reshape(36)
    t = np.ascontiguousarray(t_dual, np.float32).reshape(12)
    n = int(r3[0]) * int(r3[1]) * int(r3[2])
    out = np.zeros(4, np.float32)
    vols = np.zeros(4 * n if with_volumes else 1, np.float32)
    rc = _lib.xs_refshape_hessian(depth_dev.data_ptr(), cols * 2, rows, cols, k.ctypes.data_as(_f32p), r3.ctypes.data_as(_i32p), voxel_size,
                                  R.ctypes.data_as(_f32p), t.ctypes.data_as(_f32p), tranc_dist, gt_dev.data_ptr(), int(with_volumes),
                                  out.ctypes.data_as(_f32p), vols.ctypes.data_as(_f32p) if with_volumes else None)
    assert rc == 0
    if not with_volumes:
        return out
    return out, (vols[:n], vols[n:2 * n], vols[2 * n:3 * n], vols[3 * n:].view(np.int32))


def reference_tsdf_loss(depth_dev, rows, cols, intr4, res, voxel_size, R9, t3, tranc_dist, gt_dev, with_volumes=False):
    k = np.ascontiguousarray(intr4, np.float32)
    r3 = np.ascontiguousarray(res, np.int32)
    R = np.ascontiguousarray(R9, np.float32).reshape(9)
    t = np.ascontiguousarray(t3, np.float32).reshape(3)
    n = int(r3[0]) * int(r3[1]) * int(r3[2])
    out = np.zeros(2, np.float32)
    vols = np.zeros(2 * n if with_volumes else 1, np.float32)
    rc = _lib.xs_refshape_loss(depth_dev.data_ptr(), cols * 2, rows, cols, k.ctypes.data_as(_f32p), r3.ctypes.data_as(_i32p), voxel_size,
                               R.ctypes.data_as(_f32p), t.ctypes.data_as(_f32p), tranc_dist, gt_dev.data_ptr(), int(with_volumes),
                               out.ctypes.data_as(_f32p), vols.ctypes.data_as(_f32p) if with_volumes else None)
    assert rc == 0
    if not with_volumes:
        return out
    return out, (vols[:n], vols[n:].view(np.int32))
```

Baseline: 3963.

## Add speculative ICP launch planning, volume sign-map registry and drop per-launch syncs

Adds a launcher-state layer that records the sequence of ICP calls and speculatively queues the next expected reduction, tracks TSDF volumes in a registry so a precomputed sign/shift map can be reused or reset instead of rebuilt, and makes per-stage host synchronisation opt-in via an XS_LAUNCHERS env mode. Every device memory transfer or free now settles any queued launch and marks affected volumes dirty. The aim is to remove host-device round trips and redundant volume scans in raycast/ICP. It adds bookkeeping complexity and the risk of stale maps or wasted speculative work when call patterns diverge.

```diff
diff --git a/include/xslam_amd_pipeline.h b/include/xslam_amd_pipeline.h
--- a/include/xslam_amd_pipeline.h
+++ b/include/xslam_amd_pipeline.h
@@ -128,6 +128,25 @@
                      const float *Rv2c9, const float *tv2c3, float tranc_dist, const float *gt_dev, int with_volumes, float *out2,
                      float *volumes_host);
 
+int xs_launchers_mode(int mask);
+void xs_launchers_stats(unsigned long long *out5);
+int xs_launchers_init_volume(float *value, int *weight, float *grad, size_t vol_step, const int *res3);
+int xs_launchers_integrate(const uint16_t *depth_dev, size_t depth_step, int rows, int cols, const float *intr4, int max_weight, const int *res3,
+                           float voxel_size, const float *Rv2c18, const float *tv2c6, float tranc_dist, float *value, int *weight, float *grad,
+                           size_t vol_step, float threshold);
+int xs_launchers_raycast(const float *intr4, const float *Rc2v18, const float *tc2v6, const float *Rv2w18, const float *tv2w6, float tranc_dist,
+                         const int *res3, float voxel_size, const float *value, const float *grad, size_t vol_step, float *vmap, float *nmap,
+                         size_t map_step, int rows, int cols);
+int xs_launchers_resize_maps(const float *vmap_in, const float *nmap_in, size_t in_step, int rows, int cols, float *vmap_out, float *nmap_out,
+                             size_t out_step);
+int xs_launchers_estimate_combined(const float *Rcurr18, const float *tcurr6, const float *vmap_curr, const float *nmap_curr,
+                                   const float *Rprev_inv18, const float *tprev6, const float *intr4, const float *vmap_g_prev,
+                                   const float *nmap_g_prev, size_t map_step, int rows, int cols, float distThres, float angleThres,
+                                   double *A72_host, double *b12_host, long long *inliers);
+void xs_launchers_volume_written(const void *value);
+void xs_launchers_volume_released(const void *value);
+int xs_launchers_download(const void *dev, size_t step, int rows, int cols_bytes, void *host);
+
 #ifdef __cplusplus
 }
 #endif
diff --git a/x-slam_amd/host/device_array.hpp b/x-slam_amd/host/device_array.hpp
--- a/x-slam_amd/host/device_array.hpp
+++ b/x-slam_amd/host/device_array.hpp
@@ -1,5 +1,6 @@
 #pragma once
 #include "kernel_containers.hpp"
+#include "launcher_plan.hpp"
 #include <atomic>
 #include <cstdio>
 #include <cstdlib>
@@ -46,6 +47,8 @@
     void release() {
         if (refcount_ && refcount_->fetch_sub(1) == 1) {
             delete refcount_;
+            xs_host::settle_queued_launch();
+            xs_host::volume_released(data_);
             hipSafeCall(hipFree(data_));
         }
         data_ = nullptr; sizeBytes_ = 0; refcount_ = nullptr;
@@ -54,27 +57,35 @@
         if (empty()) other.release();
         else {
             other.create(sizeBytes_);
+            xs_host::settle_queued_launch();
+            xs_host::volume_written(other.data_);
             hipSafeCall(hipMemcpyAsync(other.data_, data_, sizeBytes_, hipMemcpyDeviceToDevice, xs_host::current_stream()));
             hipSafeCall(hipStreamSynchronize(xs_host::current_stream()));
         }
     }
     void upload(const void *host_ptr_arg, size_t sizeBytes_arg) {
         create(sizeBytes_arg);
+        xs_host::settle_queued_launch();
+        xs_host::volume_written(data_);
         hipSafeCall(hipMemcpyAsync(data_, host_ptr_arg, sizeBytes_, hipMemcpyHostToDevice, xs_host::current_stream()));
         hipSafeCall(hipStreamSynchronize(xs_host::current_stream()));
     }
     bool upload(const void *host_ptr_arg, std::size_t device_begin_byte_offset, std::size_t num_bytes) {
         if (device_begin_byte_offset + num_bytes > sizeBytes_) return false;
+        xs_host::settle_queued_launch();
+        xs_host::volume_written((char *)data_ + device_begin_byte_offset);
         hipSafeCall(hipMemcpyAsync((char *)data_ + device_begin_byte_offset, host_ptr_arg, num_bytes, hipMemcpyHostToDevice, xs_host::current_stream()));
         hipSafeCall(hipStreamSynchronize(xs_host::current_stream()));
         return true;
     }
     void download(void *host_ptr_arg) const {
+        xs_host::settle_queued_launch();
         hipSafeCall(hipMemcpyAsync(host_ptr_arg, data_, sizeBytes_, hipMemcpyDeviceToHost, xs_host::current_stream()));
         hipSafeCall(hipStreamSynchronize(xs_host::current_stream()));
     }
     bool download(void *host_ptr_arg, std::size_t device_begin_byte_offset, std::size_t num_bytes) const {
         if (device_begin_byte_offset + num_bytes > sizeBytes_) return false;
+        xs_host::settle_queued_launch();
         hipSafeCall(hipMemcpyAsync(host_ptr_arg, (const char *)data_ + device_begin_byte_offset, num_bytes, hipMemcpyDeviceToHost, xs_host::current_stream()));
         hipSafeCall(hipStreamSynchronize(xs_host::current_stream()));
         return true;
@@ -123,6 +134,8 @@
     void release() {
         if (refcount_ && refcount_->fetch_sub(1) == 1) {
             delete refcount_;
+            xs_host::settle_queued_launch();
+            xs_host::volume_released(data_);
             hipSafeCall(hipFree(data_));
         }
         colsBytes_ = 0; rows_ = 0; data_ = nullptr; step_ = 0; refcount_ = nullptr;
@@ -131,16 +144,21 @@
         if (empty()) other.release();
         else {
             other.create(rows_, colsBytes_);
+            xs_host::settle_queued_launch();
+            xs_host::volume_written(other.data_);
             hipSafeCall(hipMemcpy2DAsync(other.data_, other.step_, data_, step_, colsBytes_, rows_, hipMemcpyDeviceToDevice, xs_host::current_stream()));
             hipSafeCall(hipStreamSynchronize(xs_host::current_stream()));
         }
     }
     void upload(const void *host_ptr_arg, std::size_t host_step_arg, int rows_arg, int colsBytes_arg) {
         create(rows_arg, colsBytes_arg);
+        xs_host::settle_queued_launch();
+        xs_host::volume_written(data_);
         hipSafeCall(hipMemcpy2DAsync(data_, step_, host_ptr_arg, host_step_arg, colsBytes_, rows_, hipMemcpyHostToDevice, xs_host::current_stream()));
         hipSafeCall(hipStreamSynchronize(xs_host::current_stream()));
     }
     void download(void *host_ptr_arg, std::size_t host_step_arg) const {
+        xs_host::settle_queued_launch();
         hipSafeCall(hipMemcpy2DAsync(host_ptr_arg, host_step_arg, data_, step_, colsBytes_, rows_, hipMemcpyDeviceToHost, xs_host::current_stream()));
         hipSafeCall(hipStreamSynchronize(xs_host::current_stream()));
     }
diff --git a/x-slam_amd/host/launcher_plan.hpp b/x-slam_amd/host/launcher_plan.hpp
--- /dev/null
+++ b/x-slam_amd/host/launcher_plan.hpp
@@ -0,0 +1,195 @@
+#pragma once
+#include <cstddef>
+#include <cstdlib>
+#include <cstring>
+#include <vector>
+
+namespace xs_host {
+
+enum : int {
+    kLaunchersRefSync = 1,
+    kLaunchersNoSignMap = 2,
+    kLaunchersNoPost = 4,
+};
+inline int parse_launcher_mode(const char *text) {
+    int mode = 0;
+    for (const char *p = text ? text : ""; *p;) {
+        const char *e = p;
+        while (*e && *e != ',') ++e;
+        const size_t n = (size_t)(e - p);
+        if (n == 7 && !std::memcmp(p, "refsync", 7)) mode |= kLaunchersRefSync;
+        else if (n == 9 && !std::memcmp(p, "nosignmap", 9)) mode |= kLaunchersNoSignMap;
+        else if (n == 6 && !std::memcmp(p, "nopost", 6)) mode |= kLaunchersNoPost;
+        p = *e ? e + 1 : e;
+    }
+    return mode;
+}
+inline int &launcher_mode() { static int mode = parse_launcher_mode(std::getenv("XS_LAUNCHERS")); return mode; }
+
+struct LauncherStats {
+    unsigned long long speculated = 0;
+    unsigned long long matched = 0;
+    unsigned long long abandoned = 0;
+    unsigned long long maps_rebuilt = 0;
+    unsigned long long maps_used = 0;
+};
+
+struct IcpCall {
+    const void *vmap_curr = nullptr, *nmap_curr = nullptr, *vmap_g_prev = nullptr, *nmap_g_prev = nullptr;
+    size_t step = 0;
+    int rows = 0, cols = 0;
+    float intr[4] = {0, 0, 0, 0};
+    bool operator==(const IcpCall &o) const {
+        return vmap_curr == o.vmap_curr && nmap_curr == o.nmap_curr && vmap_g_prev == o.vmap_g_prev && nmap_g_prev == o.nmap_g_prev &&
+               step == o.step && rows == o.rows && cols == o.cols && !std::memcmp(intr, o.intr, sizeof(intr));
+    }
+    bool uses(const void *p) const { return p && (p == vmap_curr || p == nmap_curr || p == vmap_g_prev || p == nmap_g_prev); }
+};
+struct Speculated {
+    IcpCall call;
+    float Rprev_inv[18] = {0}, tprev[6] = {0};
+    float distThres = 0, angleThres = 0;
+    bool same(const Speculated &o) const {
+        return call == o.call && !std::memcmp(Rprev_inv, o.Rprev_inv, sizeof(Rprev_inv)) && !std::memcmp(tprev, o.tprev, sizeof(tprev)) &&
+               !std::memcmp(&distThres, &o.distThres, sizeof(float)) && !std::memcmp(&angleThres, &o.angleThres, sizeof(float));
+    }
+};
+struct IcpPlan {
+    std::vector<IcpCall> prev, cur;
+    bool diverged = false;
+    const IcpCall *observe(const IcpCall &c) {
+        const size_t i = cur.size();
+        cur.push_back(c);
+        if (diverged || i >= prev.size() || !(prev[i] == c)) { diverged = true; return nullptr; }
+        return i + 1 < prev.size() ? &prev[i + 1] : nullptr;
+    }
+    void end_run() {
+        if (!cur.empty()) { prev.swap(cur); cur.clear(); }
+        diverged = false;
+    }
+    void forget(const void *p) {
+        for (const IcpCall &c : prev)
+            if (c.uses(p)) { prev.clear(); break; }
+        for (const IcpCall &c : cur)
+            if (c.uses(p)) { cur.clear(); diverged = true; break; }
+    }
+};
+
+enum class MapAction { none, keep, reset, rebuild };
+struct VolumeEntry {
+    const void *value = nullptr;
+    size_t step = 0;
+    int res[3] = {0, 0, 0};
+    bool live = false;
+    bool made = false;
+    int shift = 0;
+    float voxel_size = 0, tranc_dist = 0;
+    bool dirty = false;
+    bool initialised = false;
+    bool same_key(const void *v, size_t s, const int *r) const { return value == v && step == s && res[0] == r[0] && res[1] == r[1] && res[2] == r[2]; }
+    bool holds(const void *p) const {
+        const char *b = static_cast<const char *>(value), *q = static_cast<const char *>(p);
+        return live && q >= b && q < b + step * (size_t)res[1] * (size_t)res[2];
+    }
+};
+struct VolumeRegistry {
+    std::vector<VolumeEntry> entries;
+    typedef int (*ShiftFn)(const float *intr4, float voxel_size, float tranc_dist);
+
+    int find(const void *value) const {
+        for (size_t i = 0; i < entries.size(); ++i)
+            if (entries[i].live && entries[i].value == value) return (int)i;
+        return -1;
+    }
+    int entry_for(const void *value, size_t step, const int *res) {
+        int i = find(value);
+        if (i >= 0 && entries[i].same_key(value, step, res)) return i;
+        if (i < 0) {
+            for (size_t k = 0; k < entries.size() && i < 0; ++k)
+                if (!entries[k].live) i = (int)k;
+            if (i < 0) { entries.emplace_back(); i = (int)entries.size() - 1; }
+        }
+        VolumeEntry e;
+        e.value = value; e.step = step; e.live = true;
+        std::memcpy(e.res, res, sizeof(e.res));
+        entries[i] = e;
+        return i;
+    }
+    void on_init(const void *value, size_t step, const int *res) {
+        VolumeEntry &e = entries[entry_for(value, step, res)];
+        e.initialised = true;
+        e.dirty = false;
+    }
+    MapAction on_integrate(const void *value, size_t step, const int *res, const float *intr4, float voxel_size, float tranc_dist, ShiftFn shift_of,
+                           int *index) {
+        *index = entry_for(value, step, res);
+        VolumeEntry &e = entries[*index];
+        MapAction act = MapAction::keep;
+        if (!e.made || e.voxel_size != voxel_size || e.tranc_dist != tranc_dist) {
+            e.made = true;
+            e.shift = shift_of(intr4, voxel_size, tranc_dist);
+            e.voxel_size = voxel_size; e.tranc_dist = tranc_dist;
+            act = e.initialised && !e.dirty ? MapAction::reset : MapAction::rebuild;
+        } else if (e.dirty)
+            act = MapAction::rebuild;
+        else if (e.initialised)
+            act = MapAction::reset;
+        if (e.shift == 0) {
+            e.dirty = true; e.initialised = false;
+            return MapAction::none;
+        }
+        e.dirty = false; e.initialised = false;
+        return act;
+    }
+    int on_raycast(const void *value, size_t step, const int *res, float voxel_size, float tranc_dist, int needed_shift) const {
+        const int i = find(value);
+        if (i < 0) return -1;
+        const VolumeEntry &e = entries[i];
+        if (!e.same_key(value, step, res) || !e.made || e.shift == 0 || e.dirty || e.voxel_size != voxel_size || e.tranc_dist != tranc_dist) return -1;
+        if (needed_shift == 0 || needed_shift > e.shift) return -1;
+        return i;
+    }
+    void written(const void *p) {
+        for (VolumeEntry &e : entries)
+            if (e.holds(p)) e.dirty = true;
+    }
+    void written_all() {
+        for (VolumeEntry &e : entries) e.dirty = true;
+    }
+    void released(const void *p) {
+        for (VolumeEntry &e : entries)
+            if (e.live && e.value == p) e = VolumeEntry();
+    }
+};
+
+struct LauncherState {
+    IcpPlan plan;
+    VolumeRegistry volumes;
+    LauncherStats stats;
+    void (*settle)() = nullptr;
+};
+inline bool &launcher_state_alive() { static thread_local bool alive = false; return alive; }
+struct LauncherStateHolder {
+    LauncherState s;
+    LauncherStateHolder() { launcher_state_alive() = true; }
+    ~LauncherStateHolder() { launcher_state_alive() = false; }
+};
+inline LauncherState *launcher_state() {
+    static thread_local LauncherStateHolder h;
+    return launcher_state_alive() ? &h.s : nullptr;
+}
+inline LauncherStats launcher_stats() {
+    LauncherState *s = launcher_state();
+    return s ? s->stats : LauncherStats();
+}
+inline void volume_written(const void *p) {
+    if (LauncherState *s = launcher_state()) s->volumes.written(p);
+}
+inline void volume_released(const void *p) {
+    if (LauncherState *s = launcher_state()) { s->volumes.released(p); s->plan.forget(p); }
+}
+inline void settle_queued_launch() {
+    LauncherState *s = launcher_state();
+    if (s && s->settle) s->settle();
+}
+}
diff --git a/x-slam_amd/host/launchers_capi.cpp b/x-slam_amd/host/launchers_capi.cpp
--- /dev/null
+++ b/x-slam_amd/host/launchers_capi.cpp
@@ -0,0 +1,83 @@
+#include "TsdfVolume.h"
+#include "../../include/xslam_amd_pipeline.h"
+#include <cstring>
+
+using namespace xs_host;
+
+namespace {
+MapArr map_view(const float *p, int rows, int cols, size_t step) { return MapArr(rows * 3, cols, const_cast<float *>(p), step); }
+int3 res_of(const int *r) { int3 v; v.x = r[0]; v.y = r[1]; v.z = r[2]; return v; }
+template <class T> PtrStep<T> vol_view(T *p, size_t step) { PtrStep<T> v; v.data = p; v.step = step; return v; }
+}
+
+extern "C" {
+
+int xs_launchers_mode(int mask) {
+    if (mask >= 0 && mask != launcher_mode()) {
+        settle_queued_launch();
+        if (LauncherState *s = launcher_state()) s->volumes.written_all();
+        launcher_mode() = mask & (kLaunchersRefSync | kLaunchersNoSignMap | kLaunchersNoPost);
+    }
+    return launcher_mode();
+}
+void xs_launchers_stats(unsigned long long *out5) {
+    const LauncherStats s = launcher_stats();
+    out5[0] = s.speculated; out5[1] = s.matched; out5[2] = s.abandoned; out5[3] = s.maps_rebuilt; out5[4] = s.maps_used;
+}
+int xs_launchers_init_volume(float *value, int *weight, float *grad, size_t vol_step, const int *res3) {
+    initVolume(PtrStep<short>(), vol_view(value, vol_step), vol_view(weight, vol_step), vol_view(grad, vol_step), res_of(res3));
+    return 0;
+}
+int xs_launchers_integrate(const uint16_t *depth_dev, size_t depth_step, int rows, int cols, const float *intr4, int max_weight, const int *res3,
+                           float voxel_size, const float *Rv2c18, const float *tv2c6, float tranc_dist, float *value, int *weight, float *grad,
+                           size_t vol_step, float threshold) {
+    static thread_local DeviceArray2D<float> depthScaled;
+    MatS33 R; devComplex3 t, unused = {};
+    std::memcpy(&R, Rv2c18, sizeof(R));
+    std::memcpy(&t, tv2c6, sizeof(t));
+    integrateTsdfVolume(PtrStepSz<ushort>(rows, cols, const_cast<ushort *>(depth_dev), depth_step), Intr(intr4[0], intr4[1], intr4[2], intr4[3]), max_weight,
+                        res_of(res3), voxel_size, R, t, unused, tranc_dist, vol_view(value, vol_step), vol_view(weight, vol_step), vol_view(grad, vol_step),
+                        depthScaled, 0, threshold);
+    return 0;
+}
+int xs_launchers_raycast(const float *intr4, const float *Rc2v18, const float *tc2v6, const float *Rv2w18, const float *tv2w6, float tranc_dist,
+                         const int *res3, float voxel_size, const float *value, const float *grad, size_t vol_step, float *vmap, float *nmap,
+                         size_t map_step, int rows, int cols) {
+    MatS33 Rc2v, Rv2w; devComplex3 tc2v, tv2w;
+    std::memcpy(&Rc2v, Rc2v18, sizeof(Rc2v)); std::memcpy(&tc2v, tc2v6, sizeof(tc2v));
+    std::memcpy(&Rv2w, Rv2w18, sizeof(Rv2w)); std::memcpy(&tv2w, tv2w6, sizeof(tv2w));
+    MapArr v = map_view(vmap, rows, cols, map_step), n = map_view(nmap, rows, cols, map_step);
+    raycast(Intr(intr4[0], intr4[1], intr4[2], intr4[3]), Rc2v, tc2v, Rv2w, tv2w, tranc_dist, res_of(res3), voxel_size,
+            vol_view(const_cast<float *>(value), vol_step), vol_view(const_cast<float *>(grad), vol_step), v, n);
+    return 0;
+}
+int xs_launchers_resize_maps(const float *vmap_in, const float *nmap_in, size_t in_step, int rows, int cols, float *vmap_out, float *nmap_out,
+                             size_t out_step) {
+    MapArr vi = map_view(vmap_in, rows, cols, in_step), ni = map_view(nmap_in, rows, cols, in_step);
+    MapArr vo = map_view(vmap_out, rows / 2, cols / 2, out_step), no = map_view(nmap_out, rows / 2, cols / 2, out_step);
+    resizeVMap(vi, vo);
+    resizeNMap(ni, no);
+    return 0;
+}
+int xs_launchers_estimate_combined(const float *Rcurr18, const float *tcurr6, const float *vmap_curr, const float *nmap_curr,
+                                   const float *Rprev_inv18, const float *tprev6, const float *intr4, const float *vmap_g_prev,
+                                   const float *nmap_g_prev, size_t map_step, int rows, int cols, float distThres, float angleThres,
+                                   double *A72_host, double *b12_host, long long *inliers) {
+    MatS33 Rc, Rp; devComplex3 tc, tp;
+    std::memcpy(&Rc, Rcurr18, sizeof(Rc)); std::memcpy(&tc, tcurr6, sizeof(tc));
+    std::memcpy(&Rp, Rprev_inv18, sizeof(Rp)); std::memcpy(&tp, tprev6, sizeof(tp));
+    DeviceArray2D<devComplexICP> gbuf;
+    DeviceArray<devComplexICP> mbuf;
+    estimateCombined(Rc, tc, map_view(vmap_curr, rows, cols, map_step), map_view(nmap_curr, rows, cols, map_step), Rp, tp,
+                     Intr(intr4[0], intr4[1], intr4[2], intr4[3]), map_view(vmap_g_prev, rows, cols, map_step), map_view(nmap_g_prev, rows, cols, map_step),
+                     distThres, angleThres, gbuf, mbuf, reinterpret_cast<hostComplexICP *>(A72_host), reinterpret_cast<hostComplexICP *>(b12_host), inliers);
+    return 0;
+}
+void xs_launchers_volume_written(const void *value) { volume_written(value); }
+void xs_launchers_volume_released(const void *value) { volume_released(value); }
+int xs_launchers_download(const void *dev, size_t step, int rows, int cols_bytes, void *host) {
+    DeviceMemory2D(rows, cols_bytes, const_cast<void *>(dev), step).download(host, (size_t)cols_bytes);
+    return 0;
+}
+
+}
diff --git a/x-slam_amd/host/xs_launchers.hpp b/x-slam_amd/host/xs_launchers.hpp
--- a/x-slam_amd/host/xs_launchers.hpp
+++ b/x-slam_amd/host/xs_launchers.hpp
@@ -1,5 +1,6 @@
 #pragma once
 #include "../../include/xslam_amd.h"
+#include "../csrc/xs_host_wait.h"
 #include "xs_types.hpp"
 #include "host_algebra.hpp"
 
@@ -15,7 +16,84 @@
     DeviceArray<unsigned char> icp_ws, reduce_ws, integrate_ws;
     DeviceArray<double> sums;
     DeviceArray<float> ray_ws;
+    LauncherState *state;
+    std::vector<DeviceArray<unsigned char>> maps;
+    void *mailbox = nullptr;
+    int mailbox_in_device = 0;
+    bool mailbox_tried = false;
+    void *pairs = nullptr;
+    double host_sums[64];
+    unsigned long long seq = 0;
+    bool pending = false;
+    Speculated pending_args;
+    unsigned long long pending_seq = 0;
+    unsigned pending_mail = 0;
+    float shift_key[6] = {0, 0, 0, 0, 0, 0};
+    int shift_val = -1;
+
+    Scratch() : state(launcher_state()) { if (state) state->settle = &Scratch::settle_this_thread; }
+    ~Scratch() {
+        if (launcher_state()) { abandon_pending(false); state->settle = nullptr; }
+        if (mailbox) (void)xs_icp_mailbox_free(mailbox, mailbox_in_device);
+        if (pairs) (void)hipHostFree(pairs);
+    }
     static Scratch &get() { static thread_local Scratch s; return s; }
+    static void settle_this_thread() { get().settle(); }
+    void settle() {
+        state->plan.end_run();
+        abandon_pending(true);
+    }
+    void abandon_pending(bool recover) {
+        if (!pending) return;
+        pending = false;
+        xs_icp_post_pose(mailbox, nullptr, nullptr, pending_mail, 1);
+        ++state->stats.abandoned;
+        if (recover && xs_poll_pairs(pairs, pending_seq) == xs_wait::left) reinit_icp();
+    }
+    void reinit_icp() {
+        sync();
+        check_rc(xs_icp_workspace_init(icp_ws.ptr(), current_stream()), "icp workspace");
+    }
+    bool can_post() {
+        if (!mailbox_tried) {
+            mailbox_tried = true;
+            check_rc(xs_icp_mailbox_alloc(&mailbox, &mailbox_in_device), "icp mailbox");
+            hipSafeCall(hipHostMalloc(&pairs, XS_ICP_PAIRS_BYTES, hipHostMallocCoherent | hipHostMallocMapped));
+            memset(pairs, 0, XS_ICP_PAIRS_BYTES);
+        }
+        return mailbox && mailbox_in_device && pairs;
+    }
+    unsigned long long next_seq() {
+        if ((unsigned)(seq + 1) == 0u) ++seq;
+        return ++seq;
+    }
+    int signmap_shift(const float *intr4, float voxel_size, float tranc_dist) {
+        const float key[6] = {intr4[0], intr4[1], intr4[2], intr4[3], voxel_size, tranc_dist};
+        if (shift_val < 0 || memcmp(key, shift_key, sizeof(key))) {
+            shift_val = xs_raycast_signmap_shift(intr4, voxel_size, tranc_dist);
+            memcpy(shift_key, key, sizeof(key));
+        }
+        return shift_val;
+    }
+    void *map_for_integrate(const float *value, size_t step, const int *res, const float *intr4, float voxel_size, float tranc_dist) {
+        int i = -1;
+        const MapAction act = state->volumes.on_integrate(value, step, res, intr4, voxel_size, tranc_dist, &xs_raycast_signmap_shift, &i);
+        if ((size_t)i >= maps.size()) maps.resize(i + 1);
+        if (act == MapAction::none) { maps[i].release(); return nullptr; }
+        const int shift = state->volumes.entries[i].shift;
+        const size_t bytes = xs_signmap_bytes(res, shift);
+        MapAction todo = act;
+        if (maps[i].size() != bytes) {
+            maps[i].create(bytes);
+            if (todo == MapAction::keep) todo = MapAction::rebuild;
+        }
+        if (todo == MapAction::rebuild) {
+            check_rc(xs_signmap_rebuild(maps[i].ptr(), res, shift, tranc_dist, value, step, current_stream()), "sign map rebuild");
+            ++state->stats.maps_rebuilt;
+        } else if (todo == MapAction::reset)
+            check_rc(xs_signmap_reset(maps[i].ptr(), res, shift, tranc_dist, current_stream()), "sign map reset");
+        return maps[i].ptr();
+    }
     void *icp() {
         if (icp_ws.size() != xs_icp_workspace_bytes()) {
             icp_ws.create(xs_icp_workspace_bytes());
@@ -43,8 +121,11 @@
 inline void initVolume(PtrStep<short> , PtrStep<float> value_volume,
                        PtrStep<int> weight_volume, PtrStep<float> grad_volume, const int3 &volume_resolution) {
     const int res[3] = {volume_resolution.x, volume_resolution.y, volume_resolution.z};
+    auto &S = xs_host::Scratch::get();
+    S.settle();
     xs_host::check_rc(xs_init_volume(value_volume.data, weight_volume.data, grad_volume.data, value_volume.step, res, 0, res[2],
                                      xs_host::current_stream()), "initVolume");
+    S.state->volumes.on_init(value_volume.data, value_volume.step, res);
     xs_host::sync();
 }
 
@@ -53,15 +134,22 @@
                                 float tranc_dist, PtrStep<float> value_volume, PtrStep<int> weight_volume, PtrStep<float> grad_volume,
                                 DeviceArray2D<float> &depthScaled, int , float threshold = 0.0f, float  = 0.0f,
                                 unsigned long long *updated_dev = nullptr, bool synchronise = true) {
+    auto &S = xs_host::Scratch::get();
+    S.settle();
     depthScaled.create(depth.rows, depth.cols);
     const int res[3] = {volume_resolution.x, volume_resolution.y, volume_resolution.z};
     hipStream_t st = xs_host::current_stream();
+    const int mode = xs_host::launcher_mode();
+    xs_integrate_opts o = {};
+    o.struct_bytes = sizeof(o);
+    if (mode & xs_host::kLaunchersNoSignMap) S.state->volumes.written(value_volume.data);
+    else o.signmap = S.map_for_integrate(value_volume.data, value_volume.step, res, &intr.fx, voxel_size, tranc_dist);
     xs_host::check_rc(xs_scale_depth(depth.data, depth.step, depth.rows, depth.cols, depthScaled.ptr(), depthScaled.step(), st), "scaleDepth");
-    xs_host::check_rc(xs_integrate_scaled(depthScaled.ptr(), depthScaled.step(), depth.rows, depth.cols, &intr.fx, max_weight, res, voxel_size,
-                                          &Rv2c.data[0].x.re, &tv2c.x.re, tranc_dist, value_volume.data, weight_volume.data, grad_volume.data,
-                                          value_volume.step, threshold, 0, res[2], updated_dev, nullptr, xs_host::Scratch::get().integrate(res), st),
+    xs_host::check_rc(xs_integrate_scaled_ex2(depthScaled.ptr(), depthScaled.step(), depth.rows, depth.cols, &intr.fx, max_weight, res, voxel_size,
+                                              &Rv2c.data[0].x.re, &tv2c.x.re, tranc_dist, value_volume.data, weight_volume.data, grad_volume.data,
+                                              value_volume.step, threshold, 0, res[2], updated_dev, nullptr, S.integrate(res), &o, st),
                       "integrateTsdfVolume");
-    if (synchronise) xs_host::sync();
+    if (synchronise && (mode & xs_host::kLaunchersRefSync)) xs_host::sync();
 }
 
 inline void raycast(const Intr &intr, const MatS33 &Rc2v, const devComplex3 &tc2v, const MatS33 &Rv2w, const devComplex3 &tv2w,
@@ -69,9 +157,24 @@
                     const PtrStep<float> &grad_volume, MapArr &vmap, MapArr &nmap, unsigned long long *hits_dev = nullptr,
                     float *workspace = nullptr, xs_raycast_opts *opts = nullptr) {
     const int res[3] = {volume_resolution.x, volume_resolution.y, volume_resolution.z};
+    auto &S = xs_host::Scratch::get();
+    S.settle();
+    xs_raycast_opts by_map = {};
+    if (!opts && !(xs_host::launcher_mode() & xs_host::kLaunchersNoSignMap)) {
+        const int i = S.state->volumes.on_raycast(value_volume.data, value_volume.step, res, voxel_size, tranc_dist, S.signmap_shift(&intr.fx, voxel_size, tranc_dist));
+        if (i >= 0 && (size_t)i < S.maps.size() && !S.maps[i].empty()) {
+            by_map.struct_bytes = sizeof(by_map);
+            by_map.signmap = S.maps[i].ptr();
+            by_map.signmap_shift = S.state->volumes.entries[i].shift;
+            by_map.signmap_tranc_dist = tranc_dist;
+            opts = &by_map;
+            if (!workspace) workspace = S.ray(vmap.rows() / 3, vmap.cols());
+            ++S.state->stats.maps_used;
+        }
+    }
     xs_host::check_rc(xs_raycast_ex(&intr.fx, &Rc2v.data[0].x.re, &tc2v.x.re, &Rv2w.data[0].x.re, &tv2w.x.re, tranc_dist, res, voxel_size,
                                     value_volume.data, grad_volume.data, value_volume.step, &vmap.ptr()->re, &nmap.ptr()->re, vmap.step(),
-                                    vmap.rows() / 3, vmap.cols(), hits_dev, workspace ? workspace : xs_host::Scratch::get().ray(vmap.rows() / 3, vmap.cols()), opts,
+                                    vmap.rows() / 3, vmap.cols(), hits_dev, workspace ? workspace : S.ray(vmap.rows() / 3, vmap.cols()), opts,
                                     xs_host::current_stream()), "raycast");
 }
 
@@ -80,38 +183,103 @@
                              const MapArr &nmap_g_prev, float distThres, float angleThres, DeviceArray2D<devComplexICP> & ,
                              DeviceArray<devComplexICP> & , hostComplexICP *matrixA_host, hostComplexICP *vectorB_host,
                              long long *inliers = nullptr) {
-    auto &S = xs_host::Scratch::get();
-    xs_host::check_rc(xs_estimate_combined(&Rcurr.data[0].x.re, &tcurr.x.re, &vmap_curr.ptr()->re, &nmap_curr.ptr()->re,
-                                           &Rprev_inv.data[0].x.re, &tprev.x.re, &intr.fx, &vmap_g_prev.ptr()->re, &nmap_g_prev.ptr()->re,
-                                           vmap_curr.step(), vmap_curr.rows() / 3, vmap_curr.cols(), distThres, angleThres, S.icp(),
-                                           nullptr , reinterpret_cast<double *>(matrixA_host), reinterpret_cast<double *>(vectorB_host),
-                                           inliers, xs_host::current_stream()), "estimateCombined");
+    using namespace xs_host;
+    auto &S = Scratch::get();
+    const int rows = vmap_curr.rows() / 3, cols = vmap_curr.cols();
+    hipStream_t st = current_stream();
+    if ((launcher_mode() & kLaunchersNoPost) || rows <= 0 || cols <= 0 || !S.can_post()) {
+        S.abandon_pending(true);
+        check_rc(xs_estimate_combined(&Rcurr.data[0].x.re, &tcurr.x.re, &vmap_curr.ptr()->re, &nmap_curr.ptr()->re,
+                                      &Rprev_inv.data[0].x.re, &tprev.x.re, &intr.fx, &vmap_g_prev.ptr()->re, &nmap_g_prev.ptr()->re,
+                                      vmap_curr.step(), rows, cols, distThres, angleThres, S.icp(),
+                                      nullptr , reinterpret_cast<double *>(matrixA_host), reinterpret_cast<double *>(vectorB_host),
+                                      inliers, st), "estimateCombined");
+        return;
+    }
+    Speculated now;
+    now.call.vmap_curr = vmap_curr.ptr(); now.call.nmap_curr = nmap_curr.ptr(); now.call.vmap_g_prev = vmap_g_prev.ptr(); now.call.nmap_g_prev = nmap_g_prev.ptr();
+    now.call.step = vmap_curr.step(); now.call.rows = rows; now.call.cols = cols;
+    memcpy(now.call.intr, &intr.fx, sizeof(now.call.intr));
+    memcpy(now.Rprev_inv, &Rprev_inv.data[0].x.re, sizeof(now.Rprev_inv));
+    memcpy(now.tprev, &tprev.x.re, sizeof(now.tprev));
+    now.distThres = distThres; now.angleThres = angleThres;
+    auto launch_now = [&]() {
+        const unsigned long long s = S.next_seq();
+        check_rc(xs_icp_accumulate(&Rcurr.data[0].x.re, &tcurr.x.re, &vmap_curr.ptr()->re, &nmap_curr.ptr()->re, &Rprev_inv.data[0].x.re, &tprev.x.re,
+                                   &intr.fx, &vmap_g_prev.ptr()->re, &nmap_g_prev.ptr()->re, vmap_curr.step(), rows, cols, distThres, angleThres, 0, rows,
+                                   S.icp(), static_cast<double *>(S.pairs), XS_ICP_PUBLISH_PAIRS, s, st), "estimateCombined");
+        return s;
+    };
+    unsigned long long seq;
+    const bool matched = S.pending && S.pending_args.same(now);
+    if (matched) {
+        S.pending = false;
+        xs_icp_post_pose(S.mailbox, &Rcurr.data[0].x.re, &tcurr.x.re, S.pending_mail, 0);
+        seq = S.pending_seq;
+        ++S.state->stats.matched;
+    } else {
+        S.abandon_pending(true);
+        seq = launch_now();
+    }
+    if (const IcpCall *next = S.state->plan.observe(now.call)) {
+        S.pending_args = now;
+        S.pending_args.call = *next;
+        S.pending_seq = S.next_seq();
+        S.pending_mail = (unsigned)S.pending_seq;
+        check_rc(xs_icp_accumulate_posted(S.mailbox, S.pending_mail, static_cast<const float *>(next->vmap_curr), static_cast<const float *>(next->nmap_curr),
+                                          now.Rprev_inv, now.tprev, next->intr, static_cast<const float *>(next->vmap_g_prev),
+                                          static_cast<const float *>(next->nmap_g_prev), next->step, next->rows, next->cols, distThres, angleThres, 0, next->rows,
+                                          S.icp(), static_cast<double *>(S.pairs), XS_ICP_PUBLISH_PAIRS, S.pending_seq, st), "estimateCombined (posted)");
+        S.pending = true;
+        ++S.state->stats.speculated;
+    }
+    auto wait = [&](unsigned long long s) { return xs_host_wait([&] { return xs_poll_pairs(S.pairs, s); }, 4000000000LL, st); };
+    xs_wait_result w = wait(seq);
+    if (w.status == xs_wait::left && matched) {
+        S.abandon_pending(false);
+        S.reinit_icp();
+        ++S.state->stats.abandoned;
+        w = wait(launch_now());
+    }
+    if (w.status != xs_wait::published) {
+        printf("HIP error(estimateCombined): %s\n", w.status == xs_wait::failed ? hipGetErrorString(w.error) : xs_wait_str(w.status));
+        exit(-1);
+    }
+    xs_read_pairs(S.pairs, S.host_sums);
+    xs_icp_unpack(S.host_sums, reinterpret_cast<double *>(matrixA_host), reinterpret_cast<double *>(vectorB_host));
+    if (inliers) *inliers = (long long)S.host_sums[54];
 }
 
 inline void bilateralFilter(const DeviceArray2D<ushort> &src, MapArr &dst) {
+    xs_host::Scratch::get().settle();
     xs_host::check_rc(xs_bilateral_filter(src.ptr(), src.step(), src.rows(), src.cols(), &dst.ptr()->re, dst.step(), xs_host::current_stream()), "bilateralFilter");
 }
 inline void pyrDown(const MapArr &src, MapArr &dst) {
+    xs_host::Scratch::get().settle();
     dst.create(src.rows() / 2, src.cols() / 2);
     xs_host::check_rc(xs_pyr_down(&src.ptr()->re, src.step(), src.rows(), src.cols(), &dst.ptr()->re, dst.step(), xs_host::current_stream()), "pyrDown");
 }
 inline void createVMap(const Intr &intr, const MapArr &depth, MapArr &vmap) {
+    xs_host::Scratch::get().settle();
     vmap.create(depth.rows() * 3, depth.cols());
     xs_host::check_rc(xs_create_vmap(&intr.fx, &depth.ptr()->re, depth.step(), depth.rows(), depth.cols(), &vmap.ptr()->re, vmap.step(), xs_host::current_stream()), "createVMap");
 }
 inline void createNMap(const MapArr &vmap, MapArr &nmap) {
+    xs_host::Scratch::get().settle();
     nmap.create(vmap.rows(), vmap.cols());
     xs_host::check_rc(xs_create_nmap(&vmap.ptr()->re, &nmap.ptr()->re, vmap.step(), vmap.rows() / 3, vmap.cols(), xs_host::current_stream()), "createNMap");
 }
 inline void resizeVMap(const MapArr &input, MapArr &output, bool synchronise = true) {
+    xs_host::Scratch::get().settle();
     output.create((input.rows() / 3 / 2) * 3, input.cols() / 2);
     xs_host::check_rc(xs_resize_vmap(&input.ptr()->re, input.step(), input.rows() / 3, input.cols(), &output.ptr()->re, output.step(), xs_host::current_stream()), "resizeVMap");
-    if (synchronise) xs_host::sync();
+    if (synchronise && (xs_host::launcher_mode() & xs_host::kLaunchersRefSync)) xs_host::sync();
 }
 inline void resizeNMap(const MapArr &input, MapArr &output, bool synchronise = true) {
+    xs_host::Scratch::get().settle();
     output.create((input.rows() / 3 / 2) * 3, input.cols() / 2);
     xs_host::check_rc(xs_resize_nmap(&input.ptr()->re, input.step(), input.rows() / 3, input.cols(), &output.ptr()->re, output.step(), xs_host::current_stream()), "resizeNMap");
-    if (synchronise) xs_host::sync();
+    if (synchronise && (xs_host::launcher_mode() & xs_host::kLaunchersRefSync)) xs_host::sync();
 }
 
 inline float4 ComputeLocalTsdf_hessian(const PtrStepSz<ushort> &depth, const Intr &intr, DeviceArray2D<float> &depthScaled,
@@ -119,9 +287,10 @@
                                         float tranc_dist, float , float , DeviceArray<float> &gt_vec,
                                         DeviceArray<float> &real_vec, DeviceArray<float> &grad_vec, DeviceArray<float> &hessian_vec,
                                         DeviceArray<int> &count_vec) {
+    auto &S = xs_host::Scratch::get();
+    S.settle();
     depthScaled.create(depth.rows, depth.cols);
     const int res[3] = {volume_resolution.x, volume_resolution.y, volume_resolution.z};
-    auto &S = xs_host::Scratch::get();
     hipStream_t st = xs_host::current_stream();
     xs_host::check_rc(xs_scale_depth(depth.data, depth.step, depth.rows, depth.cols, depthScaled.ptr(), depthScaled.step(), st), "scaleDepth");
     const bool vols = !real_vec.empty() && !grad_vec.empty() && !hessian_vec.empty() && !count_vec.empty();
@@ -139,9 +308,10 @@
                                      const int3 &volume_resolution, float voxel_size, const Mat33 &Rv2c, const float3 &tv2c,
                                      float tranc_dist, float , float , DeviceArray<float> &gt_vec,
                                      DeviceArray<float> &real_vec, DeviceArray<int> &count_vec) {
+    auto &S = xs_host::Scratch::get();
+    S.settle();
     depthScaled.create(depth.rows, depth.cols);
     const int res[3] = {volume_resolution.x, volume_resolution.y, volume_resolution.z};
-    auto &S = xs_host::Scratch::get();
     hipStream_t st = xs_host::current_stream();
     xs_host::check_rc(xs_scale_depth(depth.data, depth.step, depth.rows, depth.cols, depthScaled.ptr(), depthScaled.step(), st), "scaleDepth");
     const bool vols = !real_vec.empty() && !count_vec.empty();
@@ -157,6 +327,7 @@
 inline size_t extractPoints(const PtrStep<float> &value_volume, const PtrStep<int> & , const PtrStep<float> & ,
                             const int3 &volume_resolution, float voxel_size, PtrSz<float3> output, int zs0 = 0, int z0 = 0, int z1 = -1) {
     const int res[3] = {volume_resolution.x, volume_resolution.y, volume_resolution.z};
+    xs_host::Scratch::get().settle();
     static thread_local DeviceArray<unsigned char> ws;
     if (ws.size() < xs_extract_workspace_bytes(res)) ws.create(xs_extract_workspace_bytes(res));
     size_t count = 0;
@@ -168,6 +339,7 @@
 inline void extractNormals(const PtrStep<float> &value_volume, const PtrStep<int> & , const PtrStep<float> & ,
                            const int3 &volume_resolution, float voxel_size, PtrSz<float3> points, PtrSz<float3> normal, int zs0 = 0, int zs1 = -1) {
     const int res[3] = {volume_resolution.x, volume_resolution.y, volume_resolution.z};
+    xs_host::Scratch::get().settle();
     xs_host::check_rc(xs_extract_normals(value_volume.data, value_volume.step, res, voxel_size, zs0, zs1 < 0 ? res[2] : zs1,
                                          reinterpret_cast<const float *>(points.data), points.size, reinterpret_cast<float *>(normal.data),
                                          xs_host::current_stream()), "extractNormals");
diff --git a/x-slam_amd/pipeline.py b/x-slam_amd/pipeline.py
--- a/x-slam_amd/pipeline.py
+++ b/x-slam_amd/pipeline.py
@@ -111,6 +111,17 @@
     "xs_refshape_icp_log": (C.c_int, [_vp, _f64p, C.c_int]),
     "xs_refshape_hessian": (C.c_int, [_vp, _sz, C.c_int, C.c_int, _f32p, _i32p, C.c_float, _f32p, _f32p, C.c_float, _vp, C.c_int, _f32p, _f32p]),
     "xs_refshape_loss": (C.c_int, [_vp, _sz, C.c_int, C.c_int, _f32p, _i32p, C.c_float, _f32p, _f32p, C.c_float, _vp, C.c_int, _f32p, _f32p]),
+    "xs_launchers_mode": (C.c_int, [C.c_int]),
+    "xs_launchers_stats": (None, [C.POINTER(C.c_ulonglong)]),
+    "xs_launchers_init_volume": (C.c_int, [_vp, _vp, _vp, _sz, _i32p]),
+    "xs_launchers_integrate": (C.c_int, [_vp, _sz, C.c_int, C.c_int, _f32p, C.c_int, _i32p, C.c_float, _f32p, _f32p, C.c_float, _vp, _vp, _vp, _sz, C.c_float]),
+    "xs_launchers_raycast": (C.c_int, [_f32p, _f32p, _f32p, _f32p, _f32p, C.c_float, _i32p, C.c_float, _vp, _vp, _sz, _vp, _vp, _sz, C.c_int, C.c_int]),
+    "xs_launchers_resize_maps": (C.c_int, [_vp, _vp, _sz, C.c_int, C.c_int, _vp, _vp, _sz]),
+    "xs_launchers_estimate_combined": (C.c_int, [_f32p, _f32p, _vp, _vp, _f32p, _f32p, _f32p, _vp, _vp, _sz, C.c_int, C.c_int, C.c_float, C.c_float,
+                                                 _f64p, _f64p, C.POINTER(C.c_longlong)]),
+    "xs_launchers_volume_written": (None, [_vp]),
+    "xs_launchers_volume_released": (None, [_vp]),
+    "xs_launchers_download": (C.c_int, [_vp, _sz, C.c_int, C.c_int, _vp]),
 }
 for _n, (_r, _a) in _SIGS.items():
     _f = getattr(_lib, _n)
@@ -873,3 +884,69 @@
     if not with_volumes:
         return out
     return out, (vols[:n], vols[n:].view(np.int32))
+
+
+LAUNCHERS_REFSYNC, LAUNCHERS_NOSIGNMAP, LAUNCHERS_NOPOST = 1, 2, 4
+
+
+def _f32(a, n):
+    a = np.ascontiguousarray(a, np.float32).reshape(n)
+    return a, a.ctypes.data_as(_f32p)
+
+
+def launchers_mode(mask=-1):
+    return _lib.xs_launchers_mode(int(mask))
+
+
+def launchers_stats():
+    out = (C.c_ulonglong * 5)()
+    _lib.xs_launchers_stats(out)
+    return dict(zip(("speculated", "matched", "abandoned", "maps_rebuilt", "maps_used"), (int(v) for v in out)))
+
+
+def launchers_init_volume(value, weight, grad, res):
+    r3 = np.ascontiguousarray(res, np.int32)
+    assert _lib.xs_launchers_init_volume(value.data_ptr(), weight.data_ptr(), grad.data_ptr(), value.stride(0) * 4, r3.ctypes.data_as(_i32p)) == 0
+
+
+def launchers_integrate(depth_dev, rows, cols, intr4, max_weight, res, voxel_size, Rv2c, tv2c, tranc_dist, value, weight, grad, threshold=0.0):
+    r3 = np.ascontiguousarray(res, np.int32)
+    (_k, k), (_R, R), (_t, t) = _f32(intr4, 4), _f32(Rv2c, 18), _f32(tv2c, 6)
+    assert _lib.xs_launchers_integrate(depth_dev.data_ptr(), cols * 2, rows, cols, k, max_weight, r3.ctypes.data_as(_i32p), voxel_size, R, t, tranc_dist,
+                                       value.data_ptr(), weight.data_ptr(), grad.data_ptr(), value.stride(0) * 4, threshold) == 0
+
+
+def launchers_raycast(intr4, Rc2v, tc2v, Rv2w, tv2w, tranc_dist, res, voxel_size, value, grad, vmap, nmap, rows, cols):
+    r3 = np.ascontiguousarray(res, np.int32)
+    (_k, k), (_a, a), (_b, b), (_c, c), (_d, d) = _f32(intr4, 4), _f32(Rc2v, 18), _f32(tc2v, 6), _f32(Rv2w, 18), _f32(tv2w, 6)
+    assert _lib.xs_launchers_raycast(k, a, b, c, d, tranc_dist, r3.ctypes.data_as(_i32p), voxel_size, value.data_ptr(), grad.data_ptr(),
+                                     value.stride(0) * 4, vmap.data_ptr(), nmap.data_ptr(), vmap.stride(0) * 4, rows, cols) == 0
+
+
+def launchers_resize_maps(vmap_in, nmap_in, rows, cols, vmap_out, nmap_out):
+    assert _lib.xs_launchers_resize_maps(vmap_in.data_ptr(), nmap_in.data_ptr(), vmap_in.stride(0) * 4, rows, cols, vmap_out.data_ptr(), nmap_out.data_ptr(),
+                                         vmap_out.stride(0) * 4) == 0
+
+
+def launchers_estimate_combined(Rcurr, tcurr, vmap_curr, nmap_curr, Rprev_inv, tprev, intr4, vmap_g_prev, nmap_g_prev, rows, cols, dist_thres, angle_thres):
+    (_a, a), (_b, b), (_c, c), (_d, d), (_k, k) = _f32(Rcurr, 18), _f32(tcurr, 6), _f32(Rprev_inv, 18), _f32(tprev, 6), _f32(intr4, 4)
+    A, bb, inl = np.zeros(72, np.float64), np.zeros(12, np.float64), C.c_longlong(0)
+    assert _lib.xs_launchers_estimate_combined(a, b, vmap_curr.data_ptr(), nmap_curr.data_ptr(), c, d, k, vmap_g_prev.data_ptr(), nmap_g_prev.data_ptr(),
+                                               vmap_curr.stride(0) * 4, rows, cols, dist_thres, angle_thres, A.ctypes.data_as(_f64p), bb.ctypes.data_as(_f64p),
+                                               C.byref(inl)) == 0
+    return A, bb, int(inl.value)
+
+
+def launchers_volume_written(value):
+    _lib.xs_launchers_volume_written(value.data_ptr())
+
+
+def launchers_volume_released(value):
+    _lib.xs_launchers_volume_released(value.data_ptr())
+
+
+def launchers_download(t):
+    rows, row_bytes = t.shape[0], int(np.prod(t.shape[1:])) * t.element_size()
+    out = np.zeros(t.shape, {4: np.float32}[t.element_size()] if t.dtype.is_floating_point else np.int32)
+    assert _lib.xs_launchers_download(t.data_ptr(), t.stride(0) * t.element_size(), rows, row_bytes, out.ctypes.data_as(_vp)) == 0
+    return out
```

Result: no change. 3972 (median of 4 runs) (+0.2%).
